# vkit-dev/vkit-ocr-model-adaptive-scaling

Measured on AMD Instinct MI355X. Metric: images/sec fwd+bwd @1024x1024 bf16 (train step: rough+precise passes, losses, backward, clip, AdamW), higher is better.
Workload: dtype bf16

## Files before the change

### include/vkas.h

```cpp
#ifndef VKAS_H
#define VKAS_H

#include <stddef.h>
#include <stdint.h>

#ifdef __cplusplus
extern "C" {
#endif

#define VKAS_F32 0
#define VKAS_BF16 1
#define VKAS_F16 2

#define VKAS_OK 0
#define VKAS_E_ARG (-1)
#define VKAS_E_LAUNCH (-2)

#define VKAS_EPI_NONE 0
#define VKAS_EPI_GELU 1
#define VKAS_EPI_SCALE_RES 2
#define VKAS_EPI_DGELU 3
#define VKAS_EPI_ADD 4
#define VKAS_EPI_PATCH 5
#define VKAS_EPI_HEAD 6

const char* vkas_last_error(void);
int vkas_abi_version(void);

typedef struct vkas_conv_geom {
  int B, Hin, Win, Hout, Wout;
  int Cp;
  int ldx;
  int KH, KW, stride, pad;
} vkas_conv_geom;

typedef struct vkas_head_desc {
  int n_heads, pw;
  int n0[4], np[4], c[4], oc[4];
  const float* params;
  float* stats;
  float* proj;
} vkas_head_desc;

typedef struct vkas_epilogue {
  int mode;
  const float* bias;
  void* out;  long ldo;
  void* out2; long ldo2;
  const void* aux; long ldaux;
  const float* colscale;
  const float* rowscale;
  int rows_per_image;
  int patch;
  int patch_Hs, patch_Ws, patch_Cp;
  vkas_head_desc head;
} vkas_epilogue;

int vkas_pack_conv_weight(const float* w, void* out, int N, int C, int KH, int KW, int Np, int Cp, int mode,
                          int dtype, void* stream);
int vkas_pack_conv_weight_slice(const float* w, void* out, int N, int C, int KH, int KW, int Np, int Cp, int mode,
                                int n_off, int Nt, int dtype, void* stream);
int vkas_unpack_conv_wgrad(const float* gw, float* grad, int N, int C, int KH, int KW, int Np, int Cp,
                           int accumulate, void* stream);
int vkas_accumulate_many(int count, const float* const* src, float* const* dst, const int* n, void* stream);
int vkas_finalize_many(int count, const float* const* partial, const long* P, const int* n, const int* ldp,
                       float* const* out, const int* accumulate, void* stream);
long vkas_layernorm_bwd_parts(long M, int Cp);
long vkas_scale_res_bwd_parts(long M, int Cp);
long vkas_dwconv7x7_wgrad_parts(int B, int H, int W, int Cp, int dtype);
int vkas_pad_vector(const float* v, float* out, int n, int np, void* stream);
size_t vkas_dw_weight_elems(int Cp);
int vkas_pack_dw_weight(const float* w, float* out, int C, int Cp, int flip, void* stream);
int vkas_unpack_dw_wgrad(const float* gw, float* grad, int C, int Cp, int accumulate, void* stream);
int vkas_image_nchw_to_nhwc8(const float* img, void* out, int B, int C, int H, int W, int dtype, void* stream);
int vkas_nhwc_to_nchw_f32(const void* x, long ld, float* out, int B, int H, int W, int C, int dtype, void* stream);
int vkas_nchw_f32_to_nhwc(const float* g, void* out, long ld, int B, int H, int W, int C, int Cp, int dtype, void* stream);

int vkas_conv_gemm_fwd(const void* x, const vkas_conv_geom* g, const void* Bw, int Np, const vkas_epilogue* epi,
                       int dtype, void* stream);
int vkas_conv_gemm_wgrad(const void* x, const vkas_conv_geom* g, const void* dy, long lddy, int Np, float* gw,
                         float* gb, int dtype, void* stream);
int vkas_conv_gemm_wgrad_ordered(const void* x, const vkas_conv_geom* g, const void* dy, long lddy, int Np, float* gw,
                                 int dtype, void* stream);
int vkas_conv_gemm_wgrad_gelu(const void* x, const vkas_conv_geom* g, const void* dy, long lddy, int Np, float* gw,
                              float* gb, int dtype, void* stream);

size_t vkas_upconv5_fold_elems(int Np, int Cp, int f, int transposed);
int vkas_upconv5_fold(const float* w, void* out, int N, int C, int Np, int Cp, int f, int transposed, int dtype, void* stream);
int vkas_upconv5_fwd(const void* x, const vkas_conv_geom* g, int f, const void* Bf, int Np, const float* bias, void* out,
                     long ldo, int dtype, void* stream);
int vkas_upconv5_dgrad(const void* dy, long lddy, const vkas_conv_geom* g, int f, const void* Bt, int Np, void* dx, long lddx,
                       int dtype, void* stream);
size_t vkas_upconv5_wgrad_ws_bytes(int B, int H, int W, int Np);
int vkas_upconv5_wgrad(const void* x, const vkas_conv_geom* g, int f, const void* dy, long lddy, int Np, void* ws,
                       size_t ws_bytes, float* gwf, float* gb, int dtype, void* stream);
int vkas_upconv5_unfold_wgrad(const float* gwf, float* dw, int N, int C, int Np, int Cp, int f, int accumulate, void* stream);

size_t vkas_mlp_chain_image_elems(int C);
int vkas_mlp_chain_pack(const float* w1, const float* w2, const float* b1, int C, int mode, void* img, int dtype,
                        void* stream);
int vkas_mlp_chain_fwd(const void* yn, long ldyn, const void* img, const float* b2, const void* x, long ldx,
                       const float* colscale, const float* rowscale, int rows_per_image, void* h, long ldh, void* z,
                       long ldz, void* out, long ldo, long M, int C, int dtype, void* stream);
int vkas_mlp_chain_ln_fwd(const void* y, long ldy, const float* ln_gamma, const float* ln_beta, void* yn, long ldyn,
                          float* stats, const void* img, const float* b2, const void* x, long ldx, const float* colscale,
                          const float* rowscale, int rows_per_image, void* h, long ldh, void* z, long ldz, void* out,
                          long ldo, long M, int C, int dtype, void* stream);
int vkas_mlp_chain_bwd(const void* dz, long lddz, const void* img_t, const void* h, long ldh, void* dh, long lddh,
                       void* dyn, long lddyn, long M, int C, int dtype, void* stream);
int vkas_conv_gemm_tile(int wgrad, long M, int Np, int K);
int vkas_conv_gemm_kernel_id(int wgrad, const vkas_conv_geom* g, int Np, long lddy, int head_width);
typedef struct vkas_gemm_switches {
  int nt_tile, tn_tile;
  int nt_ring;
  int nt_noslab, nt_nobuf, tn_nobuf, tn_noslab, tn_no96;
} vkas_gemm_switches;
typedef struct vkas_gemm_plan_info {
  int kernel_id, family, bn, ring, buf, head, pw, nobias, xg;
  long grid_m, grid_n, tiles, splits, rows, a_bytes, b_bytes;
  unsigned grid;
  char name[44];
} vkas_gemm_plan_info;
int vkas_conv_gemm_plan(int wgrad, const vkas_conv_geom* g, int Np, long lddy, int head_width, int flags, int has_gb,
                        const vkas_gemm_switches* sw, vkas_gemm_plan_info* out);
int vkas_colsum(const void* y, long ld, long M, int Np, float* out, int accumulate, float* ws, size_t ws_bytes,
                int dtype, void* stream);
size_t vkas_colsum_ws_bytes(long M, int Np);

int vkas_dwconv7x7_fwd(const void* x, long ldx, const float* w, const float* bias, const void* addend, long ldadd,
                       void* y, long ldy, int B, int H, int W, int Cp, int dtype, void* stream);
int vkas_dwconv7x7_wgrad(const void* x, long ldx, const void* dy, long lddy, float* gw, float* gb, float* ws,
                         size_t ws_bytes, int B, int H, int W, int Cp, int dtype, void* stream);
size_t vkas_dwconv7x7_wgrad_ws_bytes(int B, int H, int W, int Cp);

int vkas_layernorm_fwd(const void* x, long ldx, const float* gamma, const float* beta, void* y, long ldy,
                       float* stats, long M, int C, int Cp, int act_gelu, int dtype, void* stream);
int vkas_layernorm_bwd(const void* x, long ldx, const float* gamma, const float* beta, const float* stats,
                       const void* dy, long lddy, void* dx, long lddx, float* dgamma, float* dbeta, float* ws,
                       size_t ws_bytes, long M, int C, int Cp, int act_gelu, int dtype, void* stream);
size_t vkas_layernorm_bwd_ws_bytes(long M, int Cp);

int vkas_pack_head_params(const float* gamma, const float* beta, const float* wproj, const float* bproj, int C, int oc,
                          int pw, float* out, void* stream);
int vkas_head_tail_fwd(const void* z, long ldz, const vkas_head_desc* hd, long M, int dtype, void* stream);
int vkas_head_rows_fwd(const void* T, const float* bias, const vkas_head_desc* hd, void* z, int B, int h, int W2, int Nt,
                       int seg_rows, int dtype, void* stream);
int vkas_head_tail_bwd(const void* z, long ldz, const vkas_head_desc* hd, const float* const* dproj, void* dz, long lddz,
                       float* dparams, float* ws, size_t ws_bytes, long M, int dtype, void* stream);
size_t vkas_head_tail_bwd_ws_bytes(long M, int pw);

int vkas_scale_res_bwd(const void* dout, long lddo, const void* z, long ldz, const float* colscale,
                       const float* rowscale, int rows_per_image, void* dz, long lddz, float* dscale, float* dbias,
                       float* ws, size_t ws_bytes, long M, int Cp, int dtype, void* stream);
size_t vkas_scale_res_bwd_ws_bytes(long M, int Cp);

int vkas_resize_fwd(const void* x, long ldx, void* y, long ldy, int B, int Hin, int Win, int Hout, int Wout,
                    int Cp, int mode, int accumulate, int dtype, void* stream);
int vkas_resize2x_x_fwd(const void* x, long ldx, void* y, long ldy, int B, int H, int Win, int Cp, int dtype, void* stream);
int vkas_resize_bwd(const void* dy, long lddy, void* dx, long lddx, int B, int Hin, int Win, int Hout, int Wout,
                    int Cp, int mode, int accumulate, int dtype, void* stream);
size_t vkas_resize_bwd_ws_bytes(int B, int Hin, int Win, int Hout, int Wout, int Cp);
int vkas_resize_bwd_ws(const void* dy, long lddy, void* dx, long lddx, float* ws, size_t ws_bytes, int B, int Hin, int Win,
                       int Hout, int Wout, int Cp, int mode, int accumulate, int dtype, void* stream);

int vkas_upconv_adj(const void* dz, long lddz, void* E, int B, int h, int w, int N, int dtype, void* stream);
size_t vkas_upconv_adj_colsum_ws_bytes(int B, int h, int w, int N);
int vkas_upconv_adj_colsum(const void* dz, long lddz, void* E, int B, int h, int w, int N, float* out, int accumulate, float* ws,
                           size_t ws_bytes, int dtype, void* stream);
int vkas_upconv_adj_colsum_seg(const void* dz, long lddz, void* E, int B, int h, int w, int N, float* out, int accumulate,
                               float* ws, size_t ws_bytes, int dtype, void* stream, int seg_rows);
int vkas_upconv_adj_unpack_wgrad(const float* gE, float* gwp, int N, int Cp, void* stream);

int vkas_adaptive_avgpool_fwd(const void* x, long ldx, void* y, long ldy, int B, int H, int W, int s, int Cp,
                              int dtype, void* stream);
int vkas_adaptive_avgpool_bwd(const void* dy, long lddy, void* dx, long lddx, int B, int H, int W, int s, int Cp,
                              int accumulate, int dtype, void* stream);

#define VKAS_PPM_MAX_BRANCHES 4
#define VKAS_PPM_MAX_SCALE 16
#define VKAS_PPM_MAX_CELLS 256
#define VKAS_PPM_MAX_C 2048
#define VKAS_PPM_MAX_CB 512
long vkas_ppm_row_groups(int B, int nb, const int* scales);
int vkas_ppm_pool_fwd(const void* x, long ldx, void* cat, long ldcat, float* rowsum, int B, int H, int W, int C, int Cb,
                      int nb, const int* scales, int dtype, void* stream);
int vkas_ppm_rows_fwd(const float* rowsum, const float* const* params, void* pooled, void* lin, float* stats, void* act, int B,
                      int H, int W, int C, int Cb, int nb, const int* scales, int dtype, void* stream);
int vkas_ppm_resize_fwd(const void* act, void* cat, long ldcat, int B, int H, int W, int C, int Cb, int nb, const int* scales,
                        int dtype, void* stream);
int vkas_ppm_resize_bwd_x(const void* dcat, long lddcat, float* tx, int B, int H, int W, int C, int Cb, int nb,
                          const int* scales, int dtype, void* stream);
int vkas_ppm_rows_bwd(const float* tx, const float* const* params, const void* lin, const float* stats, void* dz,
                      float* partial, float* dp, int B, int H, int W, int C, int Cb, int nb, const int* scales, int dtype,
                      void* stream);
int vkas_ppm_param_grads(const void* dz, const void* pooled, const float* partial, float* const* grads, const int* accumulate,
                         int B, int C, int Cb, int nb, const int* scales, int dtype, void* stream);
int vkas_ppm_pool_bwd(const void* dcat, long lddcat, const float* dp, void* dx, long lddx, int B, int H, int W, int C, int Cb,
                      int nb, const int* scales, int dtype, void* stream);

int vkas_copy_channels(const void* x, long ldx, void* y, long ldy, long M, int Cp, int accumulate, int dtype,
                       void* stream);
int vkas_copy_channel_range(const void* x, long ldx, int c_src, void* y, long ldy, int c_dst, long M, int C,
                            int zero_tail, int dtype, void* stream);
int vkas_softplus_fwd(const float* x, float* y, long n, void* stream);
int vkas_softplus_bwd(const float* x, const float* dy, float* dx, long n, void* stream);

typedef struct vkas_rough_loss_cfg {
  float focal_factor, dice_factor, l1_factor, score_min, height_min;
  float focal_alpha, focal_gamma;
  float out_scale;
} vkas_rough_loss_cfg;
int vkas_rough_loss_fwd(const float* mask_feat, const float* height_feat, const float* gt_mask,
                        const float* gt_score, int B, int H, int W, int up, int left, int CH, int CW,
                        const vkas_rough_loss_cfg* cfg, double* sums, float* loss, void* stream);
int vkas_rough_loss_bwd(const float* mask_feat, const float* height_feat, const float* gt_mask,
                        const float* gt_score, int B, int H, int W, int up, int left, int CH, int CW,
                        const vkas_rough_loss_cfg* cfg, const double* sums, const float* dloss, float* d_mask_feat,
                        float* d_height_feat, void* stream);

typedef struct vkas_precise_loss_cfg {
  float pos_l2, neg_l2, offset_l1, reg_l1, angle_ce, dist_l1, loss_factor;
  float smooth_beta;
  float out_scale;
} vkas_precise_loss_cfg;
int vkas_points_margin(const int64_t* py, const int64_t* px, long n, int H, int W, int64_t* margin, void* stream);
typedef struct vkas_precise_loss_extra_cfg {
  float mask_focal, prob_l1, prob_wahr;
  float prob_l1_beta;
  float wahr_gamma;
  float focal_alpha, focal_gamma;
} vkas_precise_loss_extra_cfg;
#define VKAS_PRECISE_LOSS_SUMS 16
int vkas_precise_loss_fwd(const float* prob, const float* offset, const float* angle, const float* dist,
                          const float* gt_score, const float* gt_mask, const int64_t* py, const int64_t* px,
                          const float* gt_offsets, const float* gt_angles, const float* gt_dists, int B, int H,
                          int W, int up, int left, int CH, int CW, int P, const vkas_precise_loss_cfg* cfg,
                          const float* mask_feat, const vkas_precise_loss_extra_cfg* ex, double* sums, float* loss,
                          void* stream);
int vkas_precise_loss_bwd(const float* prob, const float* offset, const float* angle, const float* dist,
                          const float* gt_score, const float* gt_mask, const int64_t* py, const int64_t* px,
                          const float* gt_offsets, const float* gt_angles, const float* gt_dists, int B, int H,
                          int W, int up, int left, int CH, int CW, int P, const vkas_precise_loss_cfg* cfg,
                          const float* mask_feat, const vkas_precise_loss_extra_cfg* ex, const double* sums,
                          const float* dloss, float* d_prob, float* d_offset, float* d_angle, float* d_dist,
                          float* d_mask_feat, void* stream);

#define VKAS_LOSS_FOCAL 0
#define VKAS_LOSS_DICE 1
#define VKAS_LOSS_L1 2
#define VKAS_LOSS_SMOOTH_L1 3
#define VKAS_LOSS_L2 4
#define VKAS_LOSS_WAHR 5
int vkas_elementwise_loss_fwd(int kind, const float* pred, const float* gt, const float* mask, long n, float p0, float p1,
                              float eps, double* sums, float* loss, void* stream);
int vkas_elementwise_loss_bwd(int kind, const float* pred, const float* gt, const float* mask, long n, float p0, float p1,
                              float eps, const double* sums, const float* dloss, float* dpred, void* stream);
int vkas_cross_entropy_fwd(const float* logits, const void* target, int hard, long rows, int classes, double* sums,
                           float* loss, void* stream);
int vkas_cross_entropy_bwd(const float* logits, const void* target, int hard, long rows, int classes, const float* dloss,
                           float* dlogits, void* stream);

int vkas_points_prepare(const long* py, const long* px, int B, int P, int H, int W, int* map, int* pix, long Mp, void* stream);
int vkas_points_gather_rows(const void* z, long ldz, int c0, int Ns, const float* stats, const float* const* dproj,
                            int n_heads, long M, const int* pix, long Mp, void* zs, float* stats_s, float* dproj_s,
                            int dtype, void* stream);
int vkas_points_gather_patches(const void* x, long ldx, int Cp, int B, int H, int W, const int* pix, long Mp, void* xs,
                               int dtype, void* stream);
int vkas_points_gather_patches_up2(const void* x, long ldx, int Cp, int B, int h, int w, const int* pix, long Mp, void* xs,
                                   int dtype, void* stream);
int vkas_points_scatter3x3(const float* D, const int* pix, const int* map, long Mp, int B, int H, int W, int Cp, void* dx,
                           long lddx, int dtype, void* stream);
int vkas_points_scatter3x3_low(const float* D, const int* pix, const int* map, long Mp, int B, int h, int w, int Cp, void* dx,
                               long lddx, int dtype, void* stream);

int vkas_points_scatter_vec8(const float* src, const int* pix, long Mp, float* dst, void* stream);
int vkas_points_gather_vec8(const float* src, const int* pix, long Mp, float* dst, void* stream);

typedef struct {
  const float* w;
  void* out;
  long total;
  int kind, N, C, KH, KW, Np, Cp, mode, n_off, Nt, dtype;
} vkas_pack_desc;
int vkas_pack_many(const vkas_pack_desc* descs, const int* block_start, int count, int total_blocks, void* stream);
int vkas_pack_many_blocks(const vkas_pack_desc* d);

int vkas_rough_postprocess(const float* mask_logit, const float* height, int B, int H, int W, const int* valid_h,
                           const int* valid_w, float mask_thr, float height_min, unsigned char* out_mask,
                           float* out_height, void* stream);
int vkas_precise_postprocess(const float* prob_logit, const float* offset, const float* angle, const float* dist, int B,
                             int H, int W, const int* valid_h, const int* valid_w, float* out_prob, float* out_offset,
                             float* out_angle, float* out_dist, void* stream);
long vkas_char_polygons_workspace_bytes(int B, int H, int W, int size);
int vkas_char_polygons(const float* prob, const float* offset, const float* angle, const float* dist, int B, int H, int W,
                       int size, float thr, float scale_y, float scale_x, void* workspace, size_t workspace_bytes,
                       int* count, int* points, float* probs, float* quads, void* stream);
int vkas_char_label_maps(const int* rows, const int* count, int B, int K, int h, int w, int up, int left, int CH, int CW,
                         float k, int* owner, float* mask, float* height, float* score, void* stream);
long long vkas_quad_match_workspace_bytes(int B, int M, int N, int max_pairs);
int vkas_quad_match(const int* gt_rows, const int* gt_count, const int* pred_rows, const int* pred_count, int B, int M, int N,
                    double iou_thr, int max_pairs, void* workspace, size_t workspace_bytes, int* gt_match, int* pred_match,
                    double* gt_iou, long long* stats, int* rounds, void* stream);
long long vkas_quad_match_ranked_workspace_bytes(int B, int M, int N, int T, int max_pairs);
int vkas_quad_match_ranked(const int* gt_rows, const int* gt_count, const unsigned char* gt_care, const int* pred_rows,
                           const int* pred_count, const float* probs, int B, int M, int N, const double* iou_thrs, int T,
                           double cover_thr, int max_pairs, void* workspace, size_t workspace_bytes, int* pred_match,
                           unsigned char* pred_state, int* gt_match, double* pred_iou, unsigned char* covered,
                           long long* stats, long long* dc_stats, int* rounds, void* stream);
int vkas_quad_rows(const double* quads, const unsigned char* valid, int B, int K, int* rows, void* stream);
long long vkas_quad_nms_workspace_bytes(int B, int K, int max_pairs);
int vkas_quad_nms(const int* rows, const int* count, const float* probs, int B, int K, double iou_thr, int max_pairs,
                  void* workspace, size_t workspace_bytes, unsigned char* keep, int* suppressor, long long* stats, int* rounds,
                  void* stream);
long long vkas_line_match_workspace_bytes(int B, int M, int N, int max_pairs);
int vkas_line_match(const int* gt_rows, const int* gt_count, const unsigned char* gt_care, const int* pred_rows,
                    const int* pred_count, int B, int M, int N, int tr_q8, int tp_q8, double cover_thr, int max_pairs,
                    void* workspace, size_t workspace_bytes, unsigned char* gt_kind, int* gt_group, unsigned char* pred_kind,
                    int* pred_group, long long* stats, int* rounds, void* stream);
long long vkas_ribbon_match_workspace_bytes(int B, int M, int N, int max_pairs);
int vkas_ribbon_match(const int* gt_rows, const int* gt_count, const unsigned char* gt_care, const int* gt_segs, int Sg,
                      const int* pred_rows, const int* pred_count, const int* pred_segs, int Sp, int B, int M, int N, int tr_q8,
                      int tp_q8, double cover_thr, int max_pairs, void* workspace, size_t workspace_bytes,
                      unsigned char* gt_kind, int* gt_group, unsigned char* pred_kind, int* pred_group, long long* stats,
                      int* rounds, void* stream);
long long vkas_quad_lines_workspace_bytes(int B, int K);
int vkas_quad_lines(const int* rows, const int* count, int B, int K, int gap_q4, int cross_q4, int ratio_q4, void* workspace,
                    size_t workspace_bytes, int* line, int* order, long long* table, long long* stats, void* stream);
long long vkas_text_regions_workspace_bytes(int B, int H, int W, int max_regions);
int vkas_text_regions(const unsigned char* mask, const float* height, int B, int H, int W, int max_regions, void* workspace,
                      long long workspace_bytes, int* count, int* labels, int* boxes, int* areas, int* valid, float* medians,
                      void* stream);
int vkas_resample_pack_u8(const unsigned char* src, int Hs, int Ws, const int* placements, int n, unsigned char* page,
                          int Hp, int Wp, void* stream);
int vkas_pack_region_labels(const int* labels, int Hl, int Wl, int valid_h, int valid_w, int Hs, int Ws,
                            const int* placements, const int* region_ids, int n, int fdf, int* out, int Hq, int Wq,
                            void* stream);
int vkas_resample_pack_u8_multi(const unsigned char* arena, long long arena_bytes, const long long* sources, int S,
                                const int* rows, int n, const int* page_start, unsigned char* pages, int Q, int Hp, int Wp,
                                void* stream);
int vkas_pack_region_labels_multi(const int* label_arena, long long label_words, const long long* label_sources, int S,
                                  const int* rows, int n, const int* page_start, int fdf, int* out, int Q, int Hq, int Wq,
                                  void* stream);
int vkas_region_moments(const int* labels, int B, int H, int W, int max_regions, long long* moments, void* stream);
int vkas_region_extents(const int* labels, int B, int H, int W, int max_regions, const int* dirs, int* extents,
                        void* stream);
int vkas_warp_pack_u8(const unsigned char* src, int Hs, int Ws, const long long* warps, int n, unsigned char* page, int Hp,
                      int Wp, void* stream);
int vkas_warp_region_labels(const int* labels, int Hl, int Wl, int valid_h, int valid_w, int Hs, int Ws,
                            const long long* warps, const int* region_ids, int n, int fdf, int* out, int Hq, int Wq,
                            void* stream);
int vkas_crop_warp_f32(const unsigned char* arena, long long arena_bytes, const long long* sources, int S,
                       const long long* rows, int B, float* out, int H, int W, void* stream);
int vkas_quad_strips_u8(const unsigned char* arena, long long arena_bytes, const long long* sources, int S,
                        const long long* rows, int n, int h, unsigned char* out, long long out_bytes, void* stream);
long long vkas_spine_strips_workspace_bytes(long long columns);
int vkas_spine_columns(const long long* table, int n, long long knots_total, int h, long long* columns,
                       long long columns_cap, void* stream);
int vkas_spine_strips_u8(const unsigned char* arena, long long arena_bytes, const long long* sources, int S,
                         const long long* table, int n, long long knots_total, int h, void* ws, long long ws_bytes,
                         unsigned char* out, long long out_bytes, void* stream);

int vkas_l2norm_sq(const float* g, long n, double* sumsq, void* stream);
int vkas_adamw_step(float* p, const float* g, float* m, float* v, long n, const double* sumsq, float max_norm,
                    float grad_scale, float lr, float beta1, float beta2, float eps, float weight_decay, int step,
                    void* stream);

#ifdef __cplusplus
}
#endif
#endif
```

### vkit_ocr_model_adaptive_scaling_amd/_lib.py

```python
import ctypes
import os
from ctypes import POINTER, Structure, c_char, c_char_p, c_double, c_float, c_int, c_int64, c_long, c_longlong, c_size_t, c_uint, c_void_p

_HERE = os.path.dirname(os.path.abspath(__file__))
LIB_PATH = os.environ.get('VKAS_LIB_PATH') or os.path.join(_HERE, 'libvkas.so')

F32, BF16, F16 = 0, 1, 2
EPI_NONE, EPI_GELU, EPI_SCALE_RES, EPI_DGELU, EPI_ADD, EPI_PATCH, EPI_HEAD = range(7)
LOSS_FOCAL, LOSS_DICE, LOSS_L1, LOSS_SMOOTH_L1, LOSS_L2 = range(5)
LOSS_WAHR = 5
PRECISE_LOSS_SUMS = 16


class ConvGeom(Structure):
    _fields_ = [('B', c_int), ('Hin', c_int), ('Win', c_int), ('Hout', c_int), ('Wout', c_int), ('Cp', c_int),
                ('ldx', c_int), ('KH', c_int), ('KW', c_int), ('stride', c_int), ('pad', c_int)]


class HeadDesc(Structure):
    _fields_ = [('n_heads', c_int), ('pw', c_int), ('n0', c_int * 4), ('np', c_int * 4), ('c', c_int * 4),
                ('oc', c_int * 4), ('params', c_void_p), ('stats', c_void_p), ('proj', c_void_p)]


class Epilogue(Structure):
    _fields_ = [('mode', c_int), ('bias', c_void_p), ('out', c_void_p), ('ldo', c_long), ('out2', c_void_p),
                ('ldo2', c_long), ('aux', c_void_p), ('ldaux', c_long), ('colscale', c_void_p),
                ('rowscale', c_void_p), ('rows_per_image', c_int), ('patch', c_int), ('patch_Hs', c_int),
                ('patch_Ws', c_int), ('patch_Cp', c_int), ('head', HeadDesc)]


class GemmSwitches(Structure):
    _fields_ = [('nt_tile', c_int), ('tn_tile', c_int), ('nt_ring', c_int), ('nt_noslab', c_int), ('nt_nobuf', c_int),
                ('tn_nobuf', c_int), ('tn_noslab', c_int), ('tn_no96', c_int)]

    def __init__(self, nt_ring=-1, **kw):
        super().__init__(nt_ring=nt_ring, **kw)


class GemmPlanInfo(Structure):
    _fields_ = [(n, c_int) for n in ('kernel_id', 'family', 'bn', 'ring', 'buf', 'head', 'pw', 'nobias', 'xg')] + \
               [(n, c_long) for n in ('grid_m', 'grid_n', 'tiles', 'splits', 'rows', 'a_bytes', 'b_bytes')] + \
               [('grid', c_uint), ('name', c_char * 44)]


class PackDesc(Structure):
    _fields_ = [('w', c_void_p), ('out', c_void_p), ('total', c_long), ('kind', c_int), ('N', c_int), ('C', c_int),
                ('KH', c_int), ('KW', c_int), ('Np', c_int), ('Cp', c_int), ('mode', c_int), ('n_off', c_int),
                ('Nt', c_int), ('dtype', c_int)]


class RoughLossCfg(Structure):
    _fields_ = [('focal_factor', c_float), ('dice_factor', c_float), ('l1_factor', c_float), ('score_min', c_float),
                ('height_min', c_float), ('focal_alpha', c_float), ('focal_gamma', c_float), ('out_scale', c_float)]


class PreciseLossCfg(Structure):
    _fields_ = [('pos_l2', c_float), ('neg_l2', c_float), ('offset_l1', c_float), ('reg_l1', c_float),
                ('angle_ce', c_float), ('dist_l1', c_float), ('loss_factor', c_float), ('smooth_beta', c_float),
                ('out_scale', c_float)]


class PreciseLossExtraCfg(Structure):
    _fields_ = [('mask_focal', c_float), ('prob_l1', c_float), ('prob_wahr', c_float), ('prob_l1_beta', c_float),
                ('wahr_gamma', c_float), ('focal_alpha', c_float), ('focal_gamma', c_float)]


class VkasError(RuntimeError):
    pass


if not os.path.exists(LIB_PATH):
    raise ImportError(
        f'{LIB_PATH} not found: build the HIP kernels first (python -c "import __graft_entry__ as g; g.build()" '
        f'or make -C {os.path.join(_HERE, "csrc")}).  There is no CPU fallback.')

lib = ctypes.CDLL(LIB_PATH)

_P = c_void_p
_SIGS = {
    'vkas_last_error': (c_char_p, []),
    'vkas_abi_version': (c_int, []),
    'vkas_pack_conv_weight': (c_int, [_P, _P, c_int, c_int, c_int, c_int, c_int, c_int, c_int, c_int, _P]),
    'vkas_pack_conv_weight_slice': (c_int, [_P, _P, c_int, c_int, c_int, c_int, c_int, c_int, c_int, c_int, c_int, c_int, _P]),
    'vkas_unpack_conv_wgrad': (c_int, [_P, _P, c_int, c_int, c_int, c_int, c_int, c_int, c_int, _P]),
    'vkas_accumulate_many': (c_int, [c_int, POINTER(c_void_p), POINTER(c_void_p), POINTER(c_int), _P]),
    'vkas_finalize_many': (c_int, [c_int, POINTER(c_void_p), POINTER(c_long), POINTER(c_int), POINTER(c_int), POINTER(c_void_p),
                                   POINTER(c_int), _P]),
    'vkas_layernorm_bwd_parts': (c_long, [c_long, c_int]),
    'vkas_scale_res_bwd_parts': (c_long, [c_long, c_int]),
    'vkas_dwconv7x7_wgrad_parts': (c_long, [c_int, c_int, c_int, c_int, c_int]),
    'vkas_pad_vector': (c_int, [_P, _P, c_int, c_int, _P]),
    'vkas_dw_weight_elems': (c_size_t, [c_int]),
    'vkas_pack_dw_weight': (c_int, [_P, _P, c_int, c_int, c_int, _P]),
    'vkas_unpack_dw_wgrad': (c_int, [_P, _P, c_int, c_int, c_int, _P]),
    'vkas_image_nchw_to_nhwc8': (c_int, [_P, _P, c_int, c_int, c_int, c_int, c_int, _P]),
    'vkas_nhwc_to_nchw_f32': (c_int, [_P, c_long, _P, c_int, c_int, c_int, c_int, c_int, _P]),
    'vkas_nchw_f32_to_nhwc': (c_int, [_P, _P, c_long, c_int, c_int, c_int, c_int, c_int, c_int, _P]),
    'vkas_conv_gemm_fwd': (c_int, [_P, POINTER(ConvGeom), _P, c_int, POINTER(Epilogue), c_int, _P]),
    'vkas_conv_gemm_wgrad': (c_int, [_P, POINTER(ConvGeom), _P, c_long, c_int, _P, _P, c_int, _P]),
    'vkas_conv_gemm_wgrad_ordered': (c_int, [_P, POINTER(ConvGeom), _P, c_long, c_int, _P, c_int, _P]),
    'vkas_conv_gemm_wgrad_gelu': (c_int, [_P, POINTER(ConvGeom), _P, c_long, c_int, _P, _P, c_int, _P]),
    'vkas_upconv5_fold_elems': (c_size_t, [c_int, c_int, c_int, c_int]),
    'vkas_upconv5_fold': (c_int, [_P, _P, c_int, c_int, c_int, c_int, c_int, c_int, c_int, _P]),
    'vkas_upconv5_fwd': (c_int, [_P, POINTER(ConvGeom), c_int, _P, c_int, _P, _P, c_long, c_int, _P]),
    'vkas_upconv5_dgrad': (c_int, [_P, c_long, POINTER(ConvGeom), c_int, _P, c_int, _P, c_long, c_int, _P]),
    'vkas_upconv5_wgrad_ws_bytes': (c_size_t, [c_int, c_int, c_int, c_int]),
    'vkas_upconv5_wgrad': (c_int, [_P, POINTER(ConvGeom), c_int, _P, c_long, c_int, _P, c_size_t, _P, _P, c_int, _P]),
    'vkas_upconv5_unfold_wgrad': (c_int, [_P, _P, c_int, c_int, c_int, c_int, c_int, c_int, _P]),
    'vkas_mlp_chain_image_elems': (c_size_t, [c_int]),
    'vkas_mlp_chain_pack': (c_int, [_P, _P, _P, c_int, c_int, _P, c_int, _P]),
    'vkas_mlp_chain_fwd': (c_int, [_P, c_long, _P, _P, _P, c_long, _P, _P, c_int, _P, c_long, _P, c_long, _P, c_long,
                                   c_long, c_int, c_int, _P]),
    'vkas_mlp_chain_ln_fwd': (c_int, [_P, c_long, _P, _P, _P, c_long, _P, _P, _P, _P, c_long, _P, _P, c_int, _P, c_long, _P,
                                      c_long, _P, c_long, c_long, c_int, c_int, _P]),
    'vkas_mlp_chain_bwd': (c_int, [_P, c_long, _P, _P, c_long, _P, c_long, _P, c_long, c_long, c_int, c_int, _P]),
    'vkas_conv_gemm_tile': (c_int, [c_int, c_long, c_int, c_int]),
    'vkas_conv_gemm_kernel_id': (c_int, [c_int, POINTER(ConvGeom), c_int, c_long, c_int]),
    'vkas_conv_gemm_plan': (c_int, [c_int, POINTER(ConvGeom), c_int, c_long, c_int, c_int, c_int, POINTER(GemmSwitches),
                                    POINTER(GemmPlanInfo)]),
    'vkas_colsum': (c_int, [_P, c_long, c_long, c_int, _P, c_int, _P, c_size_t, c_int, _P]),
    'vkas_colsum_ws_bytes': (c_size_t, [c_long, c_int]),
    'vkas_dwconv7x7_fwd': (c_int, [_P, c_long, _P, _P, _P, c_long, _P, c_long, c_int, c_int, c_int, c_int, c_int, _P]),
    'vkas_dwconv7x7_wgrad': (c_int, [_P, c_long, _P, c_long, _P, _P, _P, c_size_t, c_int, c_int, c_int, c_int, c_int, _P]),
    'vkas_dwconv7x7_wgrad_ws_bytes': (c_size_t, [c_int, c_int, c_int, c_int]),
    'vkas_layernorm_fwd': (c_int, [_P, c_long, _P, _P, _P, c_long, _P, c_long, c_int, c_int, c_int, c_int, _P]),
    'vkas_layernorm_bwd': (c_int, [_P, c_long, _P, _P, _P, _P, c_long, _P, c_long, _P, _P, _P, c_size_t, c_long, c_int,
                                   c_int, c_int, c_int, _P]),
    'vkas_layernorm_bwd_ws_bytes': (c_size_t, [c_long, c_int]),
    'vkas_pack_head_params': (c_int, [_P, _P, _P, _P, c_int, c_int, c_int, _P, _P]),
    'vkas_head_tail_fwd': (c_int, [_P, c_long, _P, c_long, c_int, _P]),
    'vkas_head_rows_fwd': (c_int, [_P, _P, POINTER(HeadDesc), _P, c_int, c_int, c_int, c_int, c_int, c_int, _P]),
    'vkas_resize2x_x_fwd': (c_int, [_P, c_long, _P, c_long, c_int, c_int, c_int, c_int, c_int, _P]),
    'vkas_points_gather_patches_up2': (c_int, [_P, c_long, c_int, c_int, c_int, c_int, _P, c_long, _P, c_int, _P]),
    'vkas_head_tail_bwd': (c_int, [_P, c_long, POINTER(HeadDesc), POINTER(c_void_p), _P, c_long, _P, _P, c_size_t, c_long, c_int, _P]),
    'vkas_head_tail_bwd_ws_bytes': (c_size_t, [c_long, c_int]),
    'vkas_scale_res_bwd': (c_int, [_P, c_long, _P, c_long, _P, _P, c_int, _P, c_long, _P, _P, _P, c_size_t, c_long,
                                   c_int, c_int, _P]),
    'vkas_scale_res_bwd_ws_bytes': (c_size_t, [c_long, c_int]),
    'vkas_resize_fwd': (c_int, [_P, c_long, _P, c_long, c_int, c_int, c_int, c_int, c_int, c_int, c_int, c_int, c_int, _P]),
    'vkas_resize_bwd': (c_int, [_P, c_long, _P, c_long, c_int, c_int, c_int, c_int, c_int, c_int, c_int, c_int, c_int, _P]),
    'vkas_resize_bwd_ws_bytes': (c_size_t, [c_int, c_int, c_int, c_int, c_int, c_int]),
    'vkas_resize_bwd_ws': (c_int, [_P, c_long, _P, c_long, _P, c_size_t, c_int, c_int, c_int, c_int, c_int, c_int, c_int, c_int,
                                   c_int, _P]),
    'vkas_upconv_adj': (c_int, [_P, c_long, _P, c_int, c_int, c_int, c_int, c_int, _P]),
    'vkas_upconv_adj_colsum_ws_bytes': (c_size_t, [c_int, c_int, c_int, c_int]),
    'vkas_upconv_adj_colsum': (c_int, [_P, c_long, _P, c_int, c_int, c_int, c_int, _P, c_int, _P, c_size_t, c_int, _P]),
    'vkas_upconv_adj_colsum_seg': (c_int, [_P, c_long, _P, c_int, c_int, c_int, c_int, _P, c_int, _P, c_size_t, c_int, _P, c_int]),
    'vkas_upconv_adj_unpack_wgrad': (c_int, [_P, _P, c_int, c_int, _P]),
    'vkas_adaptive_avgpool_fwd':(c_int, [_P, c_long, _P, c_long, c_int, c_int, c_int, c_int, c_int, c_int, _P]),
    'vkas_adaptive_avgpool_bwd': (c_int, [_P, c_long, _P, c_long, c_int, c_int, c_int, c_int, c_int, c_int, c_int, _P]),
    'vkas_ppm_row_groups': (c_long, [c_int, c_int, POINTER(c_int)]),
    'vkas_ppm_pool_fwd': (c_int, [_P, c_long, _P, c_long, _P] + [c_int] * 6 + [POINTER(c_int), c_int, _P]),
    'vkas_ppm_rows_fwd': (c_int, [_P, POINTER(c_void_p), _P, _P, _P, _P] + [c_int] * 6 + [POINTER(c_int), c_int, _P]),
    'vkas_ppm_resize_fwd': (c_int, [_P, _P, c_long] + [c_int] * 6 + [POINTER(c_int), c_int, _P]),
    'vkas_ppm_resize_bwd_x': (c_int, [_P, c_long, _P] + [c_int] * 6 + [POINTER(c_int), c_int, _P]),
    'vkas_ppm_rows_bwd': (c_int, [_P, POINTER(c_void_p), _P, _P, _P, _P, _P] + [c_int] * 6 + [POINTER(c_int), c_int, _P]),
    'vkas_ppm_param_grads': (c_int, [_P, _P, _P, POINTER(c_void_p), POINTER(c_int)] + [c_int] * 4 + [POINTER(c_int), c_int, _P]),
    'vkas_ppm_pool_bwd': (c_int, [_P, c_long, _P, _P, c_long] + [c_int] * 6 + [POINTER(c_int), c_int, _P]),
    'vkas_copy_channels': (c_int, [_P, c_long, _P, c_long, c_long, c_int, c_int, c_int, _P]),
    'vkas_copy_channel_range': (c_int, [_P, c_long, c_int, _P, c_long, c_int, c_long, c_int, c_int, c_int, _P]),
    'vkas_softplus_fwd': (c_int, [_P, _P, c_long, _P]),
    'vkas_softplus_bwd': (c_int, [_P, _P, _P, c_long, _P]),
    'vkas_rough_loss_fwd': (c_int, [_P, _P, _P, _P, c_int, c_int, c_int, c_int, c_int, c_int, c_int,
                                    POINTER(RoughLossCfg), _P, _P, _P]),
    'vkas_rough_loss_bwd': (c_int, [_P, _P, _P, _P, c_int, c_int, c_int, c_int, c_int, c_int, c_int,
                                    POINTER(RoughLossCfg), _P, _P, _P, _P, _P]),
    'vkas_points_margin': (c_int, [_P, _P, c_long, c_int, c_int, _P, _P]),
    'vkas_precise_loss_fwd': (c_int, [_P] * 11 + [c_int] * 8 + [POINTER(PreciseLossCfg), _P, POINTER(PreciseLossExtraCfg),
                                                                  _P, _P, _P]),
    'vkas_precise_loss_bwd': (c_int, [_P] * 11 + [c_int] * 8 + [POINTER(PreciseLossCfg), _P, POINTER(PreciseLossExtraCfg)]
                              + [_P] * 8),
    'vkas_elementwise_loss_fwd': (c_int, [c_int, _P, _P, _P, c_long, c_float, c_float, c_float, _P, _P, _P]),
    'vkas_elementwise_loss_bwd': (c_int, [c_int, _P, _P, _P, c_long, c_float, c_float, c_float, _P, _P, _P, _P]),
    'vkas_cross_entropy_fwd': (c_int, [_P, _P, c_int, c_long, c_int, _P, _P, _P]),
    'vkas_cross_entropy_bwd': (c_int, [_P, _P, c_int, c_long, c_int, _P, _P, _P]),
    'vkas_points_prepare': (c_int, [_P, _P, c_int, c_int, c_int, c_int, _P, _P, c_long, _P]),
    'vkas_points_gather_rows': (c_int, [_P, c_long, c_int, c_int, _P, _P, c_int, c_long, _P, c_long, _P, _P, _P, c_int, _P]),
    'vkas_points_gather_patches': (c_int, [_P, c_long, c_int, c_int, c_int, c_int, _P, c_long, _P, c_int, _P]),
    'vkas_points_scatter3x3': (c_int, [_P, _P, _P, c_long, c_int, c_int, c_int, c_int, _P, c_long, c_int, _P]),
    'vkas_points_scatter3x3_low': (c_int, [_P, _P, _P, c_long, c_int, c_int, c_int, c_int, _P, c_long, c_int, _P]),
    'vkas_points_scatter_vec8': (c_int, [_P, _P, c_long, _P, _P]),
    'vkas_points_gather_vec8': (c_int, [_P, _P, c_long, _P, _P]),
    'vkas_pack_many': (c_int, [_P, _P, c_int, c_int, _P]),
    'vkas_pack_many_blocks': (c_int, [_P]),
    'vkas_rough_postprocess': (c_int, [_P, _P, c_int, c_int, c_int, _P, _P, c_float, c_float, _P, _P, _P]),
    'vkas_precise_postprocess': (c_int, [_P, _P, _P, _P, c_int, c_int, c_int, _P, _P, _P, _P, _P, _P, _P]),
    'vkas_char_polygons_workspace_bytes': (c_long, [c_int, c_int, c_int, c_int]),
    'vkas_char_polygons': (c_int, [_P, _P, _P, _P, c_int, c_int, c_int, c_int, c_float, c_float, c_float, _P, c_size_t,
                                   _P, _P, _P, _P, _P]),
    'vkas_char_label_maps': (c_int, [_P, _P, c_int, c_int, c_int, c_int, c_int, c_int, c_int, c_int, c_float, _P, _P, _P, _P,
                                     _P]),
    'vkas_quad_match_workspace_bytes': (c_longlong, [c_int, c_int, c_int, c_int]),
    'vkas_quad_match': (c_int, [_P, _P, _P, _P, c_int, c_int, c_int, c_double, c_int, _P, c_size_t, _P, _P, _P, _P, _P, _P]),
    'vkas_quad_match_ranked_workspace_bytes': (c_longlong, [c_int, c_int, c_int, c_int, c_int]),
    'vkas_quad_match_ranked': (c_int, [_P, _P, _P, _P, _P, _P, c_int, c_int, c_int, _P, c_int, c_double, c_int, _P, c_size_t,
                                       _P, _P, _P, _P, _P, _P, _P, _P, _P]),
    'vkas_quad_rows': (c_int, [_P, _P, c_int, c_int, _P, _P]),
    'vkas_quad_nms_workspace_bytes': (c_longlong, [c_int, c_int, c_int]),
    'vkas_quad_nms': (c_int, [_P, _P, _P, c_int, c_int, c_double, c_int, _P, c_size_t, _P, _P, _P, _P, _P]),
    'vkas_line_match_workspace_bytes': (c_longlong, [c_int, c_int, c_int, c_int]),
    'vkas_line_match': (c_int, [_P, _P, _P, _P, _P, c_int, c_int, c_int, c_int, c_int, c_double, c_int, _P, c_size_t, _P, _P, _P,
                                _P, _P, _P, _P]),
    'vkas_ribbon_match_workspace_bytes': (c_longlong, [c_int, c_int, c_int, c_int]),
    'vkas_ribbon_match': (c_int, [_P, _P, _P, _P, c_int, _P, _P, _P, c_int, c_int, c_int, c_int, c_int, c_int, c_double, c_int,
                                  _P, c_size_t, _P, _P, _P, _P, _P, _P, _P]),
    'vkas_quad_lines_workspace_bytes': (c_longlong, [c_int, c_int]),
    'vkas_quad_lines': (c_int, [_P, _P, c_int, c_int, c_int, c_int, c_int, _P, c_size_t, _P, _P, _P, _P, _P]),
    'vkas_text_regions_workspace_bytes': (c_longlong, [c_int, c_int, c_int, c_int]),
    'vkas_text_regions': (c_int, [_P, _P, c_int, c_int, c_int, c_int, _P, c_longlong, _P, _P, _P, _P, _P, _P, _P]),
    'vkas_resample_pack_u8': (c_int, [_P, c_int, c_int, _P, c_int, _P, c_int, c_int, _P]),
    'vkas_pack_region_labels': (c_int, [_P, c_int, c_int, c_int, c_int, c_int, c_int, _P, _P, c_int, c_int, _P, c_int, c_int,
                                        _P]),
    'vkas_resample_pack_u8_multi': (c_int, [_P, c_longlong, _P, c_int, _P, c_int, _P, _P, c_int, c_int, c_int, _P]),
    'vkas_pack_region_labels_multi': (c_int, [_P, c_longlong, _P, c_int, _P, c_int, _P, c_int, _P, c_int, c_int, c_int, _P]),
    'vkas_region_moments': (c_int, [_P, c_int, c_int, c_int, c_int, _P, _P]),
    'vkas_region_extents': (c_int, [_P, c_int, c_int, c_int, c_int, _P, _P, _P]),
    'vkas_warp_pack_u8': (c_int, [_P, c_int, c_int, _P, c_int, _P, c_int, c_int, _P]),
    'vkas_warp_region_labels': (c_int, [_P, c_int, c_int, c_int, c_int, c_int, c_int, _P, _P, c_int, c_int, _P, c_int, c_int,
                                        _P]),
    'vkas_crop_warp_f32': (c_int, [_P, c_longlong, _P, c_int, _P, c_int, _P, c_int, c_int, _P]),
    'vkas_quad_strips_u8': (c_int, [_P, c_longlong, _P, c_int, _P, c_int, c_int, _P, c_longlong, _P]),
    'vkas_spine_strips_workspace_bytes': (c_longlong, [c_longlong]),
    'vkas_spine_columns': (c_int, [_P, c_int, c_longlong, c_int, _P, c_longlong, _P]),
    'vkas_spine_strips_u8': (c_int, [_P, c_longlong, _P, c_int, _P, c_int, c_longlong, c_int, _P, c_longlong, _P, c_longlong,
                                     _P]),
    'vkas_l2norm_sq':(c_int, [_P, c_long, _P, _P]),
    'vkas_adamw_step': (c_int, [_P, _P, _P, _P, c_long, _P, c_float, c_float, c_float, c_float, c_float, c_float,
                                c_float, c_int, _P]),
}

EXPORTS = tuple(_SIGS)

for _name, (_res, _args) in _SIGS.items():
    _fn = getattr(lib, _name)
    _fn.restype = _res
    _fn.argtypes = _args


def check(rc: int, what: str = ''):
    if rc != 0:
# ... 3 lines not shown
```

### vkit_ocr_model_adaptive_scaling_amd/csrc/gemm_api.hip

```cpp
#include <stdlib.h>
#include <string.h>

#include "gemm_parts.h"
#include "gemm_plan.h"

int vkas_gemm_nt_simple(const void*, const vkas_conv_geom*, const void*, int, const vkas_epilogue*, int, hipStream_t);
int vkas_gemm_tn_simple(const void*, const vkas_conv_geom*, const void*, long, int, float*, float*, int, int, hipStream_t);
int vkas_gemm_nt_mfma_bf16(const void*, const vkas_conv_geom*, const void*, int, const vkas_epilogue*, hipStream_t);
int vkas_gemm_tn_mfma_bf16(const void*, const vkas_conv_geom*, const void*, long, int, float*, float*, int, hipStream_t);
int vkas_gemm_nt_mfma_f16(const void*, const vkas_conv_geom*, const void*, int, const vkas_epilogue*, hipStream_t);
int vkas_gemm_tn_mfma_f16(const void*, const vkas_conv_geom*, const void*, long, int, float*, float*, int, hipStream_t);

static thread_local char g_err[512] = "";

void vkas_set_error(const char* fmt, ...) {
  va_list ap;
  va_start(ap, fmt);
  vsnprintf(g_err, sizeof(g_err), fmt, ap);
  va_end(ap);
}

extern "C" const char* vkas_last_error(void) { return g_err; }
extern "C" int vkas_abi_version(void) { return 1; }

// ... 60 lines not shown
  int rc = vkas_check_geom("vkas_conv_gemm_fwd", x, g, Np);
  if (rc) return rc;
  rc = vkas_check_epilogue("vkas_conv_gemm_fwd", epi, Np);
  if (rc) return rc;
  VKAS_CHECK(Bw && vkas_aligned16(Bw), "vkas_conv_gemm_fwd: weights null/misaligned");
  if (epi->mode == VKAS_EPI_PATCH)
    VKAS_CHECK((long)g->B * g->Hout * g->Wout == (long)g->B * epi->patch_Hs * epi->patch_Ws || g->B == 0,
               "vkas_conv_gemm_fwd: patch grid does not match the GEMM rows");
  if (epi->mode == VKAS_EPI_HEAD)
    VKAS_CHECK((dtype == VKAS_BF16 || dtype == VKAS_F16) && !force_simple() && (long)g->B * g->Hout * g->Wout >= 16384,
               "vkas_conv_gemm_fwd: the fused head epilogue exists for the 16-bit MFMA kernels (M >= 16384) only");
  if (g->KH == 1 && g->KW == 3)
    VKAS_CHECK((dtype == VKAS_BF16 || dtype == VKAS_F16) && !force_simple() && epi->mode == VKAS_EPI_NONE,
               "vkas_conv_gemm_fwd: the 1x3 row convolution exists for the 16-bit MFMA kernels with the plain epilogue only");
  if (dtype == VKAS_BF16 && !force_simple()) return vkas_gemm_nt_mfma_bf16(x, g, Bw, Np, epi, vkas_stream(stream));
  if (dtype == VKAS_F16 && !force_simple()) return vkas_gemm_nt_mfma_f16(x, g, Bw, Np, epi, vkas_stream(stream));
  return vkas_gemm_nt_simple(x, g, Bw, Np, epi, dtype, vkas_stream(stream));
}

extern "C" int vkas_conv_gemm_plan(int wgrad, const vkas_conv_geom* g, int Np, long lddy, int head_width, int flags, int has_gb,
                                   const vkas_gemm_switches* sw, vkas_gemm_plan_info* out) {
  VKAS_CHECK(g && out, "vkas_conv_gemm_plan: null argument");
  vkas_gemm_plan_info o = {};
  if (!sw && force_simple()) {
    snprintf(o.name, sizeof(o.name), wgrad ? "gemm_tn_simple" : "gemm_nt_simple");
  } else if (wgrad) {
    const vkas_tn_plan p = vkas_plan_tn(*g, Np, lddy, flags, has_gb != 0, sw ? *sw : *vkas_gemm_env_switches());
    o = {vkas_tn_kernel_id(p), p.family, p.tile, 0, p.buf, 0, p.pw, p.nobias, p.xg, 0, 0, p.tiles, p.splits, p.rows, p.x_bytes, p.dy_bytes, p.grid, ""};
    const char* t = p.tile == 128 ? "2,2,4" : (p.tile == 192 ? "2,4,6" : (p.tile == 224 ? "2,4,7" : "4,2,6"));
    if (p.family == VKAS_TN_SLAB) snprintf(o.name, sizeof(o.name), "conv3x3_wgrad_slab_kernel<%d>", p.tile / 16);
    else snprintf(o.name, sizeof(o.name), "gemm_tn_mfma_kernel<%s,4>", t);
  } else {
    const vkas_nt_plan p = vkas_plan_nt(*g, Np, head_width, sw ? *sw : *vkas_gemm_env_switches());
    const long tiles = p.grid_m * p.grid_n;
    o = {vkas_nt_kernel_id(p), p.family, p.bn, p.ring, p.buf, p.head, 0, 0, 0, p.grid_m, p.grid_n, tiles, 1, 0, p.a_bytes, p.b_bytes, (unsigned)tiles, ""};
    if (p.family == VKAS_NT_SLAB && p.kh == 1) snprintf(o.name, sizeof(o.name), "conv1x3_slab_mfma_kernel<%d>", p.bn / 32);
    else if (p.family == VKAS_NT_SLAB) snprintf(o.name, sizeof(o.name), "conv3x3_slab_mfma_kernel<%d,%d>", p.bn / 32, (int)p.head);
    else if (p.family == VKAS_NT_RING) snprintf(o.name, sizeof(o.name), "gemm_nt_ring_kernel<%d>", p.ring);
    else snprintf(o.name, sizeof(o.name), "gemm_nt_mfma_kernel<%s,4,%d>", p.family == VKAS_NT_REG128 ? "2,2" : "4,2", p.bn / 32);
  }
  *out = o;
  return VKAS_OK;
}

extern "C" int vkas_conv_gemm_tile(int wgrad, long M, int Np, int K) {
  if (force_simple()) return 0;
  const vkas_gemm_switches& sw = *vkas_gemm_env_switches();
  return wgrad ? vkas_tn_tile_rule(M, Np, K, sw) : vkas_nt_tile_rule(M, Np, sw);
}

extern "C" int vkas_conv_gemm_kernel_id(int wgrad, const vkas_conv_geom* g, int Np, long lddy, int head_width) {
  vkas_gemm_plan_info o;
  return g && vkas_conv_gemm_plan(wgrad, g, Np, lddy, head_width, 0, 0, nullptr, &o) == VKAS_OK ? o.kernel_id : 0;
}

static int conv_gemm_wgrad(const char* who, const void* x, const vkas_conv_geom* g, const void* dy, long lddy, int Np,
                           float* gw, float* gb, int x_gelu, int dtype, void* stream) {
  int rc = vkas_check_geom(who, x, g, Np);
  if (rc) return rc;
  VKAS_CHECK(dy && vkas_aligned16(dy) && lddy >= Np && lddy % 8 == 0, "%s: bad dy (lddy=%ld)", who, lddy);
  VKAS_CHECK(gw, "%s: null gw", who);
  VKAS_CHECK(!(g->KH == 1 && g->KW == 3), "%s: the 1x3 row convolution has no weight-gradient kernel", who);
  if (dtype == VKAS_BF16 && !force_simple())
    return vkas_gemm_tn_mfma_bf16(x, g, dy, lddy, Np, gw, gb, x_gelu, vkas_stream(stream));
  if (dtype == VKAS_F16 && !force_simple())
    return vkas_gemm_tn_mfma_f16(x, g, dy, lddy, Np, gw, gb, x_gelu, vkas_stream(stream));
  return vkas_gemm_tn_simple(x, g, dy, lddy, Np, gw, gb, x_gelu, dtype, vkas_stream(stream));
}

extern "C" int vkas_conv_gemm_wgrad(const void* x, const vkas_conv_geom* g, const void* dy, long lddy, int Np,
                                    float* gw, float* gb, int dtype, void* stream) {
  return conv_gemm_wgrad("vkas_conv_gemm_wgrad", x, g, dy, lddy, Np, gw, gb, 0, dtype, stream);
}

extern "C" int vkas_conv_gemm_wgrad_ordered(const void* x, const vkas_conv_geom* g, const void* dy, long lddy, int Np,
                                            float* gw, int dtype, void* stream) {
  return conv_gemm_wgrad("vkas_conv_gemm_wgrad_ordered", x, g, dy, lddy, Np, gw, nullptr, 2, dtype, stream);
}

extern "C" int vkas_conv_gemm_wgrad_gelu(const void* x, const vkas_conv_geom* g, const void* dy, long lddy, int Np,
                                         float* gw, float* gb, int dtype, void* stream) {
  return conv_gemm_wgrad("vkas_conv_gemm_wgrad_gelu", x, g, dy, lddy, Np, gw, gb, 1, dtype, stream);
}

namespace {
static inline long cs_rows_per_block(long M) { long r = vkas_cdiv(M > 0 ? M : 1, 1024); return r < 32 ? 32 : r; }

template <typename T>
__global__ __launch_bounds__(256) void colsum_partial_kernel(const T* __restrict__ y, long ld, long M, int Np,
                                                             long rows_per_block, float* __restrict__ partial,
                                                             int ldp) {
  const int nvec = Np >> 3;
  const int lanes_r = 256 / nvec > 0 ? 256 / nvec : 1;
  const int v = threadIdx.x % nvec;
  const int rl = threadIdx.x / nvec;
  float acc[8] = {0, 0, 0, 0, 0, 0, 0, 0};
  const long mbeg = (long)blockIdx.x * rows_per_block;
  const long mend = mbeg + rows_per_block < M ? mbeg + rows_per_block : M;
  if (rl < lanes_r) {
    for (long m = mbeg + rl; m < mend; m += lanes_r) {
      float t[8];
      load8(y + m * ld + v * 8, t);
#pragma unroll
      for (int i = 0; i < 8; ++i) acc[i] += t[i];
    }
  }
  __shared__ float red[256 * 8];
#pragma unroll
  for (int i = 0; i < 8; ++i) red[threadIdx.x * 8 + i] = acc[i];
  __syncthreads();
  if (rl == 0) {
    for (int r = 1; r < lanes_r; ++r)
#pragma unroll
      for (int i = 0; i < 8; ++i) acc[i] += red[(r * nvec + v) * 8 + i];
    float* dst = partial + (long)blockIdx.x * ldp + v * 8;
#pragma unroll
    for (int i = 0; i < 8; ++i) dst[i] = acc[i];
  }
}
}

__global__ __launch_bounds__(256) void vkas_colreduce_finalize_kernel(const float* __restrict__ partial, long P, int n,
                                                                      int ldp, float* __restrict__ out,
                                                                      int accumulate) {
  __shared__ float red[16][17];
  const int cl = threadIdx.x & 15, rl = threadIdx.x >> 4;
  const int c = blockIdx.x * 16 + cl;
  float acc[8];
#pragma unroll
  for (int i = 0; i < 8; ++i) acc[i] = 0.f;
  if (c < n) {
    long p = rl;
    for (; p + 7 * 16 < P; p += 8 * 16) {
#pragma unroll
      for (int i = 0; i < 8; ++i) acc[i] += partial[(p + 16 * i) * ldp + c];
    }
    for (; p < P; p += 16) acc[0] += partial[p * ldp + c];
  }
  red[rl][cl] = ((acc[0] + acc[1]) + (acc[2] + acc[3])) + ((acc[4] + acc[5]) + (acc[6] + acc[7]));
  __syncthreads();
  if (rl == 0 && c < n) {
    float s = 0.f;
#pragma unroll
    for (int r = 0; r < 16; ++r) s += red[r][cl];
    out[c] = accumulate ? out[c] + s : s;
  }
}

struct FinalizeMany {
  const float* partial[8];
  float* out[8];
  long P[8];
  int n[8], ldp[8], accumulate[8], first[9];
};
__global__ __launch_bounds__(256) void vkas_finalize_many_kernel(FinalizeMany a) {
  __shared__ float red[16][17];
  int k = 0;
#pragma unroll
  for (int i = 1; i < 8; ++i) k += ((int)blockIdx.x >= a.first[i]) ? 1 : 0;
  const float* __restrict__ partial = a.partial[k];
  const long P = a.P[k];
  const int n = a.n[k], ldp = a.ldp[k];
  const int cl = threadIdx.x & 15, rl = threadIdx.x >> 4;
  const int c = ((int)blockIdx.x - a.first[k]) * 16 + cl;
  float acc[8];
#pragma unroll
  for (int i = 0; i < 8; ++i) acc[i] = 0.f;
  if (c < n) {
    long p = rl;
    for (; p + 7 * 16 < P; p += 8 * 16) {
#pragma unroll
      for (int i = 0; i < 8; ++i) acc[i] += partial[(p + 16 * i) * ldp + c];
    }
    for (; p < P; p += 16) acc[0] += partial[p * ldp + c];
  }
  red[rl][cl] = ((acc[0] + acc[1]) + (acc[2] + acc[3])) + ((acc[4] + acc[5]) + (acc[6] + acc[7]));
  __syncthreads();
  if (rl == 0 && c < n) {
    float s = 0.f;
#pragma unroll
    for (int r = 0; r < 16; ++r) s += red[r][cl];
    float* out = a.out[k];
    out[c] = a.accumulate[k] ? out[c] + s : s;
  }
}

extern "C" int vkas_finalize_many(int count, const float* const* partial, const long* P, const int* n, const int* ldp,
                                  float* const* out, const int* accumulate, void* stream) {
  VKAS_CHECK(count >= 0 && count <= 8 && (count == 0 || (partial && P && n && ldp && out && accumulate)),
             "vkas_finalize_many: bad arguments (count=%d)", count);
  if (count == 0) return VKAS_OK;
  FinalizeMany a;
  int blocks = 0;
  for (int k = 0; k < 8; ++k) {
    a.first[k] = blocks;
    if (k < count) {
      VKAS_CHECK(partial[k] && out[k] && P[k] >= 0 && n[k] >= 0 && ldp[k] >= n[k], "vkas_finalize_many: bad reduction %d", k);
      a.partial[k] = partial[k];
      a.out[k] = out[k];
      a.P[k] = P[k];
      a.n[k] = n[k];
      a.ldp[k] = ldp[k];
      a.accumulate[k] = accumulate[k];
      blocks += (int)vkas_cdiv(n[k], 16);
    } else {
      a.partial[k] = nullptr; a.out[k] = nullptr; a.P[k] = 0; a.n[k] = 0; a.ldp[k] = 0; a.accumulate[k] = 0;
    }
  }
  a.first[8] = blocks;
  for (int k = count; k < 8; ++k) a.first[k] = blocks;
  if (blocks == 0) return VKAS_OK;
  vkas_finalize_many_kernel<<<(unsigned)blocks, 256, 0, vkas_stream(stream)>>>(a);
  VKAS_LAUNCH_CHECK("finalize_many");
  return VKAS_OK;
}

int vkas_colreduce_finalize(const float* partial, long P, int n, int ldp, float* out, int accumulate,
                            hipStream_t st) {
  vkas_colreduce_finalize_kernel<<<(unsigned)vkas_cdiv(n, 16), 256, 0, st>>>(partial, P, n, ldp, out, accumulate);
  VKAS_LAUNCH_CHECK("colreduce_finalize");
  return VKAS_OK;
}

extern "C" size_t vkas_colsum_ws_bytes(long M, int Np) {
  return (size_t)vkas_cdiv(M > 0 ? M : 1, cs_rows_per_block(M)) * (size_t)Np * sizeof(float);
}

extern "C" int vkas_colsum(const void* y, long ld, long M, int Np, float* out, int accumulate, float* ws,
                           size_t ws_bytes, int dtype, void* stream) {
  VKAS_CHECK(y && out && ws, "vkas_colsum: null pointer");
  VKAS_CHECK(Np > 0 && Np % 8 == 0, "vkas_colsum: Np=%d must be a positive multiple of 8", Np);
  VKAS_CHECK(ld >= Np && ld % 8 == 0 && vkas_aligned16(y), "vkas_colsum: bad ld/alignment");
  VKAS_CHECK(ws_bytes >= vkas_colsum_ws_bytes(M, Np), "vkas_colsum: workspace too small");
  if (M <= 0) {
    if (!accumulate) (void)hipMemsetAsync(out, 0, Np * sizeof(float), vkas_stream(stream));
    return VKAS_OK;
  }
  const long rpb = cs_rows_per_block(M);
  const long P = vkas_cdiv(M, rpb);
  VKAS_DISPATCH_DTYPE(dtype, "vkas_colsum", {
    for (int c0 = 0; c0 < Np; c0 += 2048) {
      const int n = Np - c0 < 2048 ? Np - c0 : 2048;
      colsum_partial_kernel<T><<<(unsigned)P, 256, 0, vkas_stream(stream)>>>((const T*)y + c0, ld, M, n, rpb, ws + c0, Np);
    }
  })
  VKAS_LAUNCH_CHECK("colsum_partial");
  return vkas_colreduce_finalize(ws, P, Np, Np, out, accumulate, vkas_stream(stream));
}
```

### vkit_ocr_model_adaptive_scaling_amd/csrc/mlp_chain.hip

```cpp
#include <stdlib.h>

#include <type_traits>

#include "vkas_common.h"

namespace {

typedef __attribute__((address_space(3))) void* lds_void_ptr;

constexpr int MODE_FWD = 0, MODE_BWD = 1;

#ifndef CHAIN_ABL
#define CHAIN_ABL 0
#endif
constexpr int ABL = CHAIN_ABL;

__host__ __device__ constexpr int chain_ka(int KS) { return ((KS + 1) / 2) * 64; }
__host__ __device__ constexpr int chain_img_elems(int KS) { return 32 * chain_ka(KS) + KS * 32 * 32 + 512; }

template <typename T, typename V4>
__device__ __forceinline__ V4 chain_gelu4(const V4& h) {
  const f32x2 a = gelu2_t<T>(f32x2{(float)h[0], (float)h[1]}), b = gelu2_t<T>(f32x2{(float)h[2], (float)h[3]});
  V4 o;
  o[0] = (T)a.x; o[1] = (T)a.y; o[2] = (T)b.x; o[3] = (T)b.y;
  return o;
}
template <typename T, typename V4>
__device__ __forceinline__ V4 chain_dgelu4(const V4& h, const f32x4& d) {
  const f32x2 a = f32x2{d[0], d[1]} * dgelu2_t<T>(f32x2{(float)h[0], (float)h[1]});
  const f32x2 b = f32x2{d[2], d[3]} * dgelu2_t<T>(f32x2{(float)h[2], (float)h[3]});
  V4 o;
  o[0] = (T)a.x; o[1] = (T)a.y; o[2] = (T)b.x; o[3] = (T)b.y;
  return o;
}

template <typename T>
__global__ void mlp_chain_pack_kernel(const float* __restrict__ w1, const float* __restrict__ w2,
                                      const float* __restrict__ b1, int C, int HID, int KS, int mode, T* __restrict__ img) {
  const int KA = chain_ka(KS);
  const int pieces = chain_img_elems(KS) / 8;
  const long idx = (long)blockIdx.x * blockDim.x + threadIdx.x;
  const int nchunks = HID / 32;
  if (idx >= (long)nchunks * pieces) return;
  const int j = (int)(idx / pieces);
  int p = (int)(idx - (long)j * pieces);
  float v[8];
  const int a_pieces = 32 * KA / 8;
  const int b_pieces = KS * 32 * 32 / 8;
  if (p >= a_pieces + b_pieces) {
    const int q = p - a_pieces - b_pieces;
    float4 bv = make_float4(0.f, 0.f, 0.f, 0.f);
    if (q < 8 && mode == 0 && b1) bv = *reinterpret_cast<const float4*>(b1 + j * 32 + q * 4);
    *reinterpret_cast<float4*>(img + idx * 8) = bv;
    return;
  }
  if (p < a_pieces) {
    const int s = p / 256, rem = p - s * 256;
    const int h = rem >> 3, cpos = rem & 7;
    const int c = cpos ^ (h & 7);
    const int k0 = s * 64 + c * 8;
    const int hid = j * 32 + h;
#pragma unroll
    for (int i = 0; i < 8; ++i) {
      const int k = k0 + i;
      v[i] = k < C ? (mode == 0 ? w1[(long)hid * C + k] : w2[(long)k * HID + hid]) : 0.f;
    }
  } else {
    p -= a_pieces;
    const int R = p >> 3, cpos = p & 7;
    const int c = cpos ^ (R & 7);
    const int n = R * 2 + (c >> 2), g = c & 3;
#pragma unroll
    for (int q = 0; q < 8; ++q) {
      const int hid = j * 32 + (q >> 2) * 16 + g * 4 + (q & 3);
      v[q] = n < C ? (mode == 0 ? w2[(long)n * HID + hid] : w1[(long)hid * C + n]) : 0.f;
    }
  }
  store8(img + idx * 8, v);
}

struct ChainArgs {
  const void* a;
  long lda;
  const void* img;
  void* mid_out;
  long ldm;
  const void* mid_in;
  long ldmi;
  const float* bias_b;
  const void* res;
  long ldres;
  const float* colscale;
  const float* rowscale;
  int rows_per_image;
  void* z;
  long ldz;
  void* out;
  long ldo;
  long M;
  int C, HID;
  const float* ln_gamma;
  const float* ln_beta;
  void* ln_out;
  long ldln;
  float* ln_stats;
};

template <typename T> struct Frag;
template <> struct Frag<bf16_t> { typedef bf16x8 v8; typedef bf16x4 v4; };
template <> struct Frag<f16_t> { typedef f16x8 v8; typedef f16x4 v4; };

__device__ __forceinline__ f32x4 mfma16(bf16x8 a, bf16x8 b, f32x4 c) {
  return __builtin_amdgcn_mfma_f32_16x16x32_bf16(a, b, c, 0, 0, 0);
}
__device__ __forceinline__ f32x4 mfma16(f16x8 a, f16x8 b, f32x4 c) {
  return __builtin_amdgcn_mfma_f32_16x16x32_f16(a, b, c, 0, 0, 0);
}

template <int NTHR>
__device__ __forceinline__ void chain_layernorm_stage(const ChainArgs& p, float* lnp, int tid) {
  const int cq = p.C >> 2;
  for (int i = tid; i < 2 * cq; i += NTHR) {
    const bool hi = i >= cq;
    const int idx = hi ? i - cq : i;
    *reinterpret_cast<float4*>(lnp + (hi ? p.C : 0) + idx * 4) = *reinterpret_cast<const float4*>((hi ? p.ln_beta : p.ln_gamma) + idx * 4);
  }
}

template <typename T, int TM, int KS, typename V8, typename RowFn>
__device__ __forceinline__ void chain_layernorm_rows(V8 (&xf)[TM][KS], const ChainArgs& p, RowFn mrow, int g, const float* lnp) {
  const int C = p.C;
  float mean[TM], rstd[TM];
#pragma unroll
  for (int i = 0; i < TM; ++i) {
    float s = 0.f;
#pragma unroll
    for (int ks = 0; ks < KS; ++ks)
#pragma unroll
      for (int e = 0; e < 8; ++e) s += (float)xf[i][ks][e];
    s += __shfl_xor(s, 16, 64);
    s += __shfl_xor(s, 32, 64);
    mean[i] = s / (float)C;
    float q = 0.f;
#pragma unroll
    for (int ks = 0; ks < KS; ++ks) {
      if (ks * 32 + g * 8 < C) {
#pragma unroll
        for (int e = 0; e < 8; ++e) {
          const float d = (float)xf[i][ks][e] - mean[i];
          q += d * d;
        }
      }
    }
    q += __shfl_xor(q, 16, 64);
    q += __shfl_xor(q, 32, 64);
    rstd[i] = rsqrtf(q / (float)C + 1e-6f);
  }
  T* Y = reinterpret_cast<T*>(p.ln_out);
#pragma unroll
  for (int ks = 0; ks < KS; ++ks) {
    const int k = ks * 32 + g * 8;
    const bool k_ok = k < C;
    float gv[8], bv[8];
    load8(lnp + (k_ok ? k : 0), gv);
    load8(lnp + C + (k_ok ? k : 0), bv);
#pragma unroll
    for (int i = 0; i < TM; ++i) {
      const long m = mrow(i);
      const bool ok = k_ok && m < p.M;
      V8 o;
#pragma unroll
      for (int e = 0; e < 8; ++e) o[e] = ok ? (T)(((float)xf[i][ks][e] - mean[i]) * rstd[i] * gv[e] + bv[e]) : (T)0.f;
      xf[i][ks] = o;
      if (Y && ok) *reinterpret_cast<V8*>(Y + m * p.ldln + k) = o;
    }
  }
  if (p.ln_stats && g == 0) {
#pragma unroll
    for (int i = 0; i < TM; ++i) {
      const long m = mrow(i);
      if (m < p.M) {
        p.ln_stats[2 * m] = mean[i];
        p.ln_stats[2 * m + 1] = rstd[i];
      }
    }
  }
}

template <typename T, int KS, int TM, int MODE, int MINB>
__global__ __launch_bounds__(256, MINB) void mlp_chain_kernel(ChainArgs p) {
  typedef typename Frag<T>::v8 v8;
  typedef typename Frag<T>::v4 v4;
  constexpr int NT2 = 2 * KS;
#ifdef CHAIN_OLD_SCHED
  constexpr bool HOIST = false;
#else
  constexpr bool HOIST = KS >= 4;
#endif
  constexpr int KA = chain_ka(KS);
  constexpr int IMG = chain_img_elems(KS);
  constexpr int NI = IMG * 2 / 1024;
  constexpr int ROWS = TM * 16;
  constexpr int STG = ROWS * 64;
  constexpr int NF = ROWS / 8;
  constexpr int PE = KS * 32 + 8;
  constexpr int LDS_MAIN = 2 * IMG + 4 * STG, LDS_EPI = 4 * ROWS * PE;
  constexpr int LDS_ELEMS = LDS_MAIN > LDS_EPI ? LDS_MAIN : LDS_EPI;
  static_assert((IMG * 2) % 1024 == 0, "chunk image must be whole 1-KB DMA pieces");
  __shared__ __attribute__((aligned(1024))) T lds[LDS_ELEMS];
  typedef __attribute__((address_space(3))) T lds_T;
  const int tid = threadIdx.x;
  const int lane = tid & 63;
  const int wave = __builtin_amdgcn_readfirstlane(tid >> 6);
  const int fr = lane & 15, g = lane >> 4;
  const int C = p.C;
  const long row0 = ((long)blockIdx.x * 4 + wave) * ROWS;
  const int nchunks = p.HID / 32;
  const bool full_rows = row0 + ROWS <= p.M;
  const int n_img = (NI - wave + 3) / 4;
  constexpr unsigned OOB = 0xFFFFFFF0u;

#ifdef CHAIN_BUILTIN_DMA
  const __amdgpu_buffer_rsrc_t rs_w =
      __builtin_amdgcn_make_buffer_rsrc((void*)p.img, (short)0, (int)((long)nchunks * IMG * 2), 0x00020000);
#else
  const u32x4 rs_w = vkas_make_rsrc(p.img, (unsigned)((long)nchunks * IMG * 2));
  const unsigned lds0 = vkas_lds_addr(lds);
#endif
  auto issue_chunk = [&](int j, int buf) {
#pragma unroll
    for (int q = 0; q < (NI + 3) / 4; ++q) {
// ... 600 lines not shown
        __builtin_amdgcn_sched_barrier(0);
      }
    }
    if constexpr (HAS_A) {
#pragma unroll
      for (int ab = 0; ab < NB_A; ++ab) {
        if (ab + 1 < NB_A) read_a(ab + 1, (S0 + ab + 1) & 1);
        __builtin_amdgcn_sched_barrier(0);
        mul_a(ab, (S0 + ab) & 1);
        __builtin_amdgcn_sched_barrier(0);
      }
    }
  };

  auto chunk = [&](auto no_b_c, int j) __attribute__((always_inline)) {
    constexpr bool NO_B = decltype(no_b_c)::value;
    std::integral_constant<bool, !NO_B> first_c;
    CHAIN_TR(0);
    if constexpr (CHAIN_PRIO == 1) __builtin_amdgcn_s_setprio(1);
    mfma_phase(first_c, std::true_type{}, j - 1, j);
    if constexpr (CHAIN_PRIO == 1) __builtin_amdgcn_s_setprio(0);
    CHAIN_TR(1);
    if (grp == 1) asm volatile("s_waitcnt vmcnt(0)" ::: "memory");
    asm volatile("s_waitcnt lgkmcnt(0)" ::: "memory");
    CHAIN_TR(2);
    __builtin_amdgcn_s_barrier();
    asm volatile("" ::: "memory");
    CHAIN_TR(3);
    if constexpr (CHAIN_PRIO == 2) __builtin_amdgcn_s_setprio(1);
    if (grp == 1) {
      if (!(ABL & 16)) {
        if (j + 2 < nchunks) issue_a(j + 2, wq, 4);
        if (j + 1 < nchunks) issue_b(j + 1, wq, 4);
      }
      if constexpr (MODE == MODE_BWD) {
        if ((j & 1) == 0 && j >= 2 && (j >> 1) + 1 < (nchunks + 1) / 2 && !(ABL & 1)) issue_h((j >> 1) + 1);
      }
    } else if (keep_mid && !(ABL & 1) && (j & 1) == 0 && j >= 2) {
      flush_pair((j >> 1) - 1, 64);
    }
    {
      const int e0 = (j & 1) * 32 + g * 4;
      T* stg = stg_base((j >> 1) & 1);
#pragma unroll
      for (int i = 0; i < TM; ++i) {
        const int r = (t * TM + i) * 16 + fr;
        v4 h0, h1;
        if constexpr (MODE == MODE_FWD) {
          h0[0] = (T)d[i][0][0]; h0[1] = (T)d[i][0][1]; h0[2] = (T)d[i][0][2]; h0[3] = (T)d[i][0][3];
          h1[0] = (T)d[i][1][0]; h1[1] = (T)d[i][1][1]; h1[2] = (T)d[i][1][2]; h1[3] = (T)d[i][1][3];
          if (keep_mid) {
            *reinterpret_cast<v4*>(stg + stg_off(r, e0)) = h0;
            *reinterpret_cast<v4*>(stg + stg_off(r, e0 + 16)) = h1;
          }
          const v4 g0 = (ABL & 4) ? h0 : chain_gelu4<T, v4>(h0), g1 = (ABL & 4) ? h1 : chain_gelu4<T, v4>(h1);
#pragma unroll
          for (int q = 0; q < 4; ++q) {
            own[i][q] = g0[q];
            own[i][4 + q] = g1[q];
          }
        } else {
          h0 = hq[i][0];
          h1 = hq[i][1];
          v4 o0, o1;
          if constexpr ((ABL & 4) != 0) {
#pragma unroll
            for (int q = 0; q < 4; ++q) {
              o0[q] = (T)(d[i][0][q] * (float)h0[q]);
              o1[q] = (T)(d[i][1][q] * (float)h1[q]);
            }
          } else {
            o0 = chain_dgelu4<T, v4>(h0, d[i][0]);
            o1 = chain_dgelu4<T, v4>(h1, d[i][1]);
          }
#pragma unroll
          for (int q = 0; q < 4; ++q) {
            own[i][q] = o0[q];
            own[i][4 + q] = o1[q];
          }
          *reinterpret_cast<v4*>(stg + stg_off(r, e0)) = o0;
          *reinterpret_cast<v4*>(stg + stg_off(r, e0 + 16)) = o1;
        }
        *reinterpret_cast<v8*>(exch_at(j & 1, t, i)) = own[i];
      }
    }
    if constexpr (CHAIN_PRIO == 2) __builtin_amdgcn_s_setprio(0);
    asm volatile("s_waitcnt lgkmcnt(0)" ::: "memory");
    CHAIN_TR(4);
    __builtin_amdgcn_s_barrier();
    asm volatile("" ::: "memory");
    CHAIN_TR(5);
  };
  chunk(std::true_type{}, 0);
  for (int j = 1; j < nchunks; ++j) chunk(std::false_type{}, j);
  mfma_phase(std::true_type{}, std::false_type{}, nchunks - 1, -1);
  asm volatile("s_waitcnt lgkmcnt(0)" ::: "memory");
  if (grp == 0) {
    __builtin_amdgcn_s_barrier();
    asm volatile("" ::: "memory");
    if (keep_mid && !(ABL & 1)) flush_pair((nchunks - 1) >> 1, (nchunks & 1) ? 32 : 64);
    asm volatile("s_waitcnt lgkmcnt(0)" ::: "memory");
  }
  __builtin_amdgcn_s_barrier();
  asm volatile("" ::: "memory");

  T* ep = lds + wave * (RP * PE);
  const int col0 = t * KS * 16;
#pragma unroll
  for (int n = 0; n < KS; ++n) {
    const int col = n * 16 + g * 4;
    float4 b2 = make_float4(0.f, 0.f, 0.f, 0.f);
    if constexpr (MODE == MODE_FWD) {
      if (col0 + col < C) b2 = *reinterpret_cast<const float4*>(p.bias_b + col0 + col);
    }
#pragma unroll
    for (int i = 0; i < RG; ++i) {
      v4 zq;
      zq[0] = (T)(acc[i][n][0] + b2.x);
      zq[1] = (T)(acc[i][n][1] + b2.y);
      zq[2] = (T)(acc[i][n][2] + b2.z);
      zq[3] = (T)(acc[i][n][3] + b2.w);
      *reinterpret_cast<v4*>(ep + (i * 16 + fr) * PE + col) = zq;
    }
  }
  constexpr int PCS = KS * 2;
  constexpr int RPI = 64 / PCS;
  const int piece = lane % PCS, rsub = lane / PCS;
  const int gcol = col0 + piece * 8;
  if (rsub < RPI && gcol < C) {
    float cs[8];
#pragma unroll
    for (int q = 0; q < 8; ++q) cs[q] = 0.f;
    if constexpr (MODE == MODE_FWD) load8(p.colscale + gcol, cs);
#pragma unroll 4
    for (int r = rsub; r < RP; r += RPI) {
      const long m = row0 + r;
      if (m >= p.M) break;
      const v8 zq = *reinterpret_cast<const v8*>(ep + r * PE + piece * 8);
      if constexpr (MODE == MODE_FWD) {
        if (p.z) *reinterpret_cast<v8*>(reinterpret_cast<T*>(p.z) + m * p.ldz + gcol) = zq;
        const float rs = p.rowscale ? p.rowscale[(int)(m / p.rows_per_image)] : 1.0f;
        float xr[8];
        load8(reinterpret_cast<const T*>(p.res) + m * p.ldres + gcol, xr);
#pragma unroll
        for (int q = 0; q < 8; ++q) xr[q] += rs * cs[q] * (float)zq[q];
        store8(reinterpret_cast<T*>(p.out) + m * p.ldo + gcol, xr);
      } else {
        *reinterpret_cast<v8*>(reinterpret_cast<T*>(p.out) + m * p.ldo + gcol) = zq;
      }
    }
  }
}

static int chain_ks(int C) {
  if (C <= 0 || C % 8 != 0 || C > 512) return 0;
  const int ks = (C + 31) / 32;
  return ks <= 4 ? ks : (ks <= 6 ? 6 : (ks <= 8 ? 8 : (ks <= 12 ? 12 : 16)));
}

static int chain_pair_mode() {
  static const int mode = [] {
    const char* v = getenv("VKAS_CHAIN_PAIR");
    return (v && v[0] == '0') ? 0 : 1;
  }();
  return mode;
}

template <typename T, int MODE>
static int launch_chain(const ChainArgs& a, hipStream_t st) {
  const int ks = chain_ks(a.C);
#define VKAS_CHAIN(KSV, TMV, MINB)                                                                \
  {                                                                                               \
    const long rows_per_block = 4L * TMV * 16;                                                    \
    const unsigned grid = (unsigned)vkas_cdiv(a.M, rows_per_block);                               \
    mlp_chain_kernel<T, KSV, TMV, MODE, MINB><<<grid, 256, 0, st>>>(a);                           \
  }
  switch (ks) {
    case 1: VKAS_CHAIN(1, 4, 2) break;
    case 2: VKAS_CHAIN(2, 4, 2) break;
    case 3: VKAS_CHAIN(3, 4, 2) break;
    case 4: VKAS_CHAIN(4, 2, 2) break;
    case 6: VKAS_CHAIN(6, 2, 2) break;
    case 8: VKAS_CHAIN(8, 2, 1) break;
    case 12:
      if (a.C % 16 == 0 && chain_pair_mode() != 0) {
        const unsigned grid = (unsigned)vkas_cdiv(a.M, 128);
        mlp_chain_pair_kernel<T, 12, 1, MODE><<<grid, 512, 0, st>>>(a);
      } else {
        VKAS_CHAIN(12, 2, 1)
      }
      break;
    case 16: VKAS_CHAIN(16, 2, 1) break;
    default:
      vkas_set_error("vkas_mlp_chain: C=%d is not covered (multiple of 8, <= 512)", a.C);
      return VKAS_E_ARG;
  }
#undef VKAS_CHAIN
  return VKAS_OK;
}

}

extern "C" size_t vkas_mlp_chain_image_elems(int C) {
  const int ks = chain_ks(C);
  return ks ? (size_t)(4 * C / 32) * (size_t)chain_img_elems(ks) : 0;
}

extern "C" int vkas_mlp_chain_pack(const float* w1, const float* w2, const float* b1, int C, int mode, void* img, int dtype,
                                   void* stream) {
  VKAS_CHECK(w1 && w2 && img && vkas_aligned16(img) && (mode != 0 || (b1 && vkas_aligned16(b1))),
             "vkas_mlp_chain_pack: null / misaligned pointer");
  const int ks = chain_ks(C);
  VKAS_CHECK(ks > 0, "vkas_mlp_chain_pack: C=%d is not covered (multiple of 8, <= 512)", C);
  VKAS_CHECK(mode == 0 || mode == 1, "vkas_mlp_chain_pack: mode must be 0 (forward) or 1 (backward)");
  VKAS_CHECK(dtype == VKAS_BF16 || dtype == VKAS_F16, "vkas_mlp_chain_pack: 16-bit storage types only");
  const long pieces = (long)(4 * C / 32) * (chain_img_elems(ks) / 8);
  if (dtype == VKAS_BF16)
    mlp_chain_pack_kernel<bf16_t><<<(unsigned)vkas_cdiv(pieces, 256), 256, 0, vkas_stream(stream)>>>(w1, w2, b1, C, 4 * C, ks,
                                                                                                     mode, (bf16_t*)img);
  else
    mlp_chain_pack_kernel<f16_t><<<(unsigned)vkas_cdiv(pieces, 256), 256, 0, vkas_stream(stream)>>>(w1, w2, b1, C, 4 * C, ks,
                                                                                                    mode, (f16_t*)img);
  VKAS_LAUNCH_CHECK("mlp_chain_pack");
  return VKAS_OK;
}

static int chain_check_act(const char* who, const void* p, long ld, int width) {
  VKAS_CHECK(p && vkas_aligned16(p) && ld >= width && ld % 8 == 0, "%s: bad activation operand (ld=%ld, width=%d)", who, ld, width);
  return VKAS_OK;
}

static int chain_fwd_impl(const char* who, const void* yn, long ldyn, const float* ln_gamma, const float* ln_beta, void* ln_out, long ldln,
                          float* ln_stats, const void* img, const float* b2, const void* x, long ldx, const float* colscale,
                          const float* rowscale, int rows_per_image, void* h, long ldh, void* z, long ldz, void* out, long ldo,
                          long M, int C, int dtype, void* stream) {
  VKAS_CHECK(dtype == VKAS_BF16 || dtype == VKAS_F16, "%s: 16-bit storage types only", who);
  VKAS_CHECK(chain_ks(C) > 0, "%s: C=%d is not covered (multiple of 8, <= 512)", who, C);
  VKAS_CHECK(img && b2 && colscale && vkas_aligned16(img) && vkas_aligned16(b2) && vkas_aligned16(colscale),
             "%s: null / misaligned parameter", who);
  VKAS_CHECK(M >= 0 && rows_per_image > 0, "%s: bad sizes", who);
  int rc;
  if ((rc = chain_check_act(who, yn, ldyn, C)) || (rc = chain_check_act(who, x, ldx, C)) || (rc = chain_check_act(who, out, ldo, C)))
    return rc;
  VKAS_CHECK((h == nullptr) == (z == nullptr), "%s: h and z must be given (training) or omitted (inference) together", who);
  if (h && ((rc = chain_check_act(who, h, ldh, 4 * C)) || (rc = chain_check_act(who, z, ldz, C)))) return rc;
  if (M == 0) return VKAS_OK;
  ChainArgs a = {};
  a.a = yn; a.lda = ldyn; a.img = img; a.mid_out = h; a.ldm = ldh; a.bias_b = b2; a.res = x; a.ldres = ldx;
  a.colscale = colscale; a.rowscale = rowscale; a.rows_per_image = rows_per_image; a.z = z; a.ldz = ldz; a.out = out; a.ldo = ldo;
  a.M = M; a.C = C; a.HID = 4 * C;
  a.ln_gamma = ln_gamma; a.ln_beta = ln_beta; a.ln_out = ln_out; a.ldln = ldln; a.ln_stats = ln_stats;
  rc = dtype == VKAS_BF16 ? launch_chain<bf16_t, MODE_FWD>(a, vkas_stream(stream))
                          : launch_chain<f16_t, MODE_FWD>(a, vkas_stream(stream));
  if (rc) return rc;
  VKAS_LAUNCH_CHECK("mlp_chain_fwd");
  return VKAS_OK;
}

extern "C" int vkas_mlp_chain_fwd(const void* yn, long ldyn, const void* img, const float* b2, const void* x, long ldx, const float* colscale, const float* rowscale, int rows_per_image, void* h, long ldh,
                                  void* z, long ldz, void* out, long ldo, long M, int C, int dtype, void* stream) {
  return chain_fwd_impl("vkas_mlp_chain_fwd", yn, ldyn, nullptr, nullptr, nullptr, 0, nullptr, img, b2, x, ldx, colscale, rowscale,
                        rows_per_image, h, ldh, z, ldz, out, ldo, M, C, dtype, stream);
}

extern "C" int vkas_mlp_chain_ln_fwd(const void* y, long ldy, const float* ln_gamma, const float* ln_beta, void* yn, long ldyn,
                                     float* stats, const void* img, const float* b2, const void* x, long ldx,
                                     const float* colscale, const float* rowscale, int rows_per_image, void* h, long ldh, void* z,
                                     long ldz, void* out, long ldo, long M, int C, int dtype, void* stream) {
  const char* who = "vkas_mlp_chain_ln_fwd";
  VKAS_CHECK(ln_gamma && ln_beta && vkas_aligned16(ln_gamma) && vkas_aligned16(ln_beta), "%s: null / misaligned LayerNorm parameter", who);
  VKAS_CHECK((yn == nullptr) == (h == nullptr) && (stats == nullptr) == (h == nullptr),
             "%s: yn and stats must be given (training) or omitted (inference) together with h and z", who);
  if (yn) {
    VKAS_CHECK(vkas_aligned16(yn) && ldyn >= C && ldyn % 8 == 0, "%s: bad activation operand yn (ld=%ld, width=%d)", who, ldyn, C);
  }
  return chain_fwd_impl(who, y, ldy, ln_gamma, ln_beta, yn, ldyn, stats, img, b2, x, ldx, colscale, rowscale, rows_per_image, h, ldh,
                        z, ldz, out, ldo, M, C, dtype, stream);
}

extern "C" int vkas_mlp_chain_bwd(const void* dz, long lddz, const void* img_t, const void* h, long ldh, void* dh, long lddh,
                                  void* dyn, long lddyn, long M, int C, int dtype, void* stream) {
  const char* who = "vkas_mlp_chain_bwd";
  VKAS_CHECK(dtype == VKAS_BF16 || dtype == VKAS_F16, "%s: 16-bit storage types only", who);
  VKAS_CHECK(chain_ks(C) > 0, "%s: C=%d is not covered (multiple of 8, <= 512)", who, C);
  VKAS_CHECK(img_t && vkas_aligned16(img_t) && M >= 0, "%s: bad arguments", who);
  int rc;
  if ((rc = chain_check_act(who, dz, lddz, C)) || (rc = chain_check_act(who, h, ldh, 4 * C)) || (rc = chain_check_act(who, dh, lddh, 4 * C)) ||
      (rc = chain_check_act(who, dyn, lddyn, C)))
    return rc;
  if (M == 0) return VKAS_OK;
  ChainArgs a = {};
  a.a = dz; a.lda = lddz; a.img = img_t; a.mid_out = dh; a.ldm = lddh; a.mid_in = h; a.ldmi = ldh; a.out = dyn; a.ldo = lddyn;
  a.M = M; a.C = C; a.HID = 4 * C;
  rc = dtype == VKAS_BF16 ? launch_chain<bf16_t, MODE_BWD>(a, vkas_stream(stream))
                          : launch_chain<f16_t, MODE_BWD>(a, vkas_stream(stream));
  if (rc) return rc;
  VKAS_LAUNCH_CHECK("mlp_chain_bwd");
  return VKAS_OK;
}

#ifdef CHAIN_TRACE
extern "C" int vkas_chain_trace_read(void* dst, size_t bytes) {
  return (int)hipMemcpyFromSymbol(dst, HIP_SYMBOL(vkas_chain_trace_buf), bytes < sizeof(vkas_chain_trace_buf) ? bytes : sizeof(vkas_chain_trace_buf));
}
#endif
```

### vkit_ocr_model_adaptive_scaling_amd/csrc/pack.hip

```cpp
#include "vkas_common.h"

namespace {

__device__ __forceinline__ float pack_conv_elem(const float* __restrict__ w, long i, int N, int C, int KH, int KW, int Np, int Cp,
                                                int mode, int n_off, int Nt, long& o) {
  int n, c, ky, kx;
  long r = i;
  o = i;
  if (mode == 0) {
    c = (int)(r % Cp); r /= Cp;
    kx = (int)(r % KW); r /= KW;
    ky = (int)(r % KH); r /= KH;
    n = (int)r;
    o = i + (long)n_off * KH * KW * Cp;
  } else if (mode == 1) {
    n = (int)(r % Np); r /= Np;
    o = r * Nt + n_off + n;
    kx = KW - 1 - (int)(r % KW); r /= KW;
    ky = KH - 1 - (int)(r % KH); r /= KH;
    c = (int)r;
  } else if (mode == 3) {
    c = (int)(r % Cp); r /= Cp;
    kx = (int)(r % KW); r /= KW;
    ky = (int)(r % KH); r /= KH;
    n = (int)r;
    o = (((long)ky * Nt + n_off + n) * KW + kx) * Cp + c;
  } else {
    n = (int)(r % Np); r /= Np;
    c = (int)(r % Cp); r /= Cp;
    kx = (int)(r % KW); r /= KW;
    ky = (int)r;
  }
  return (n < N && c < C) ? w[(((long)n * C + c) * KH + ky) * KW + kx] : 0.f;
}

__device__ __forceinline__ bool pack_dw_elem(const float* __restrict__ w, int i, int C, int Cp, int flip, float& v) {
  if (i < 49 * Cp) {
    const int tap = i / Cp, c = i - tap * Cp;
    const int src_tap = flip ? 48 - tap : tap;
    v = c < C ? w[(long)c * 49 + src_tap] : 0.f;
    return true;
  }
  const int j = i - 49 * Cp;
  if (j >= (Cp / 2) * 112) return false;
  const int p = j / 112, r = j - p * 112;
  const int ky = r >> 4, e = r & 15;
  const int kx = e >> 1, c = 2 * p + (e & 1);
  v = 0.f;
  if (kx < 7 && c < C) {
    const int tap = ky * 7 + kx;
    v = w[(long)c * 49 + (flip ? 48 - tap : tap)];
  }
  return true;
}

constexpr int PM_ELEMS = 2048;
__global__ __launch_bounds__(256) void pack_many_kernel(const vkas_pack_desc* __restrict__ descs,
                                                        const int* __restrict__ block_start, int count) {
  int lo = 0, hi = count;
  while (hi - lo > 1) {
    const int mid = (lo + hi) >> 1;
    if ((int)blockIdx.x >= block_start[mid]) lo = mid;
    else hi = mid;
  }
  const vkas_pack_desc d = descs[lo];
  const int lb = (int)blockIdx.x - block_start[lo];
  if (d.kind == 0 && d.mode == 1) {
    __shared__ float tile[64][33];
    const int KHW = d.KH * d.KW, J = d.C * KHW, Jp = d.Cp * KHW;
    const int tiles_n = (d.Np + 63) >> 6;
    const int jo0 = (lb / tiles_n) * 32, n0 = (lb % tiles_n) * 64;
    {
      const int l = threadIdx.x & 31, r = threadIdx.x >> 5;
      const int jo = jo0 + l;
      const int c = jo / KHW, tap = KHW - 1 - (jo - c * KHW);
      const bool j_ok = jo < Jp && c < d.C;
#pragma unroll
      for (int rr = 0; rr < 8; ++rr) {
        const int nl = rr * 8 + r, n = n0 + nl;
        tile[nl][l] = (j_ok && n < d.N) ? d.w[(long)n * J + c * KHW + tap] : 0.f;
      }
    }
    __syncthreads();
    const int l2 = threadIdx.x & 63, r2 = threadIdx.x >> 6;
    const int n = n0 + l2;
#pragma unroll
    for (int k = 0; k < 8; ++k) {
      const int row = k * 4 + r2, jo = jo0 + row;
      if (jo < Jp && n < d.Np) {
        const long o = (long)jo * d.Nt + d.n_off + n;
        const float v = tile[l2][row];
        if (d.dtype == VKAS_BF16) reinterpret_cast<bf16_t*>(d.out)[o] = from_f32<bf16_t>(v);
        else if (d.dtype == VKAS_F16) reinterpret_cast<f16_t*>(d.out)[o] = from_f32<f16_t>(v);
        else reinterpret_cast<float*>(d.out)[o] = v;
      }
    }
    return;
  }
  const long base = (long)lb * PM_ELEMS;
#pragma unroll
  for (int u = 0; u < PM_ELEMS / 256; ++u) {
    const long i = base + u * 256 + threadIdx.x;
    if (i >= d.total) return;
    if (d.kind == 1) {
      float v;
      if (pack_dw_elem(d.w, (int)i, d.C, d.Cp, d.mode, v)) reinterpret_cast<float*>(d.out)[i] = v;
    } else {
      long o;
      const float v = pack_conv_elem(d.w, i, d.N, d.C, d.KH, d.KW, d.Np, d.Cp, d.mode, d.n_off, d.Nt, o);
      if (d.dtype == VKAS_BF16) reinterpret_cast<bf16_t*>(d.out)[o] = from_f32<bf16_t>(v);
      else if (d.dtype == VKAS_F16) reinterpret_cast<f16_t*>(d.out)[o] = from_f32<f16_t>(v);
      else reinterpret_cast<float*>(d.out)[o] = v;
    }
  }
}

template <typename T>
__global__ void pack_conv_weight_kernel(const float* __restrict__ w, T* __restrict__ out, int N, int C, int KH, int KW,
                                        int Np, int Cp, int mode, long total, int n_off, int Nt) {
  for (long i = (long)blockIdx.x * blockDim.x + threadIdx.x; i < total; i += (long)gridDim.x * blockDim.x) {
    long o2;
    const float v2 = pack_conv_elem(w, i, N, C, KH, KW, Np, Cp, mode, n_off, Nt, o2);
    out[o2] = from_f32<T>(v2);
  }
}

__global__ void unpack_conv_wgrad_kernel(const float* __restrict__ gw, float* __restrict__ grad, int N, int C, int KH,
                                         int KW, int Np, int Cp, int accumulate, long total) {
  for (long i = (long)blockIdx.x * blockDim.x + threadIdx.x; i < total; i += (long)gridDim.x * blockDim.x) {
    long r = i;
    const int kx = (int)(r % KW); r /= KW;
    const int ky = (int)(r % KH); r /= KH;
    const int c = (int)(r % C); r /= C;
    const int n = (int)r;
    const float v = gw[(((long)n * KH + ky) * KW + kx) * Cp + c];
    grad[i] = accumulate ? grad[i] + v : v;
  }
}

__global__ void pad_vector_kernel(const float* __restrict__ v, float* __restrict__ out, int n, int np) {
  const int i = blockIdx.x * blockDim.x + threadIdx.x;
  if (i < np) out[i] = i < n ? v[i] : 0.f;
}

__global__ void pack_dw_weight_kernel(const float* __restrict__ w, float* __restrict__ out, int C, int Cp, int flip) {
  const int i = blockIdx.x * blockDim.x + threadIdx.x;
  float pv;
  if (pack_dw_elem(w, i, C, Cp, flip, pv)) out[i] = pv;
}

__global__ void unpack_dw_wgrad_kernel(const float* __restrict__ gw, float* __restrict__ grad, int C, int Cp,
                                       int accumulate) {
  const int i = blockIdx.x * blockDim.x + threadIdx.x;
  if (i >= C * 49) return;
  const int c = i / 49, tap = i - c * 49;
  const float v = gw[(long)tap * Cp + c];
  grad[i] = accumulate ? grad[i] + v : v;
}

template <typename T>
__global__ void image_to_nhwc8_kernel(const float* __restrict__ img, T* __restrict__ out, int B, int C, int H, int W) {
  const long total = (long)B * H * W;
  for (long p = (long)blockIdx.x * blockDim.x + threadIdx.x; p < total; p += (long)gridDim.x * blockDim.x) {
    const long hw = (long)H * W;
    const int b = (int)(p / hw);
    const long r = p - (long)b * hw;
    float v[8] = {0, 0, 0, 0, 0, 0, 0, 0};
    for (int c = 0; c < C; ++c) v[c] = img[((long)b * C + c) * hw + r];
    store8(out + p * 8, v);
  }
}

template <typename T>
__global__ void nhwc_to_nchw_kernel(const T* __restrict__ x, long ld, float* __restrict__ out, int B, long HW, int C) {
  const long total = (long)B * C * HW;
  for (long i = (long)blockIdx.x * blockDim.x + threadIdx.x; i < total; i += (long)gridDim.x * blockDim.x) {
    const long r = i % HW;
    const long bc = i / HW;
    const int c = (int)(bc % C);
    const long b = bc / C;
    out[i] = to_f32(x[(b * HW + r) * ld + c]);
  }
}

template <typename T>
__global__ void nchw_to_nhwc_kernel(const float* __restrict__ g, T* __restrict__ out, long ld, int B, long HW, int C,
                                    int Cp) {
  const long total = (long)B * HW * Cp;
  for (long i = (long)blockIdx.x * blockDim.x + threadIdx.x; i < total; i += (long)gridDim.x * blockDim.x) {
    const int c = (int)(i % Cp);
    const long p = i / Cp;
    const long b = p / HW;
    const long r = p - b * HW;
    const float v = c < C ? g[(b * C + c) * HW + r] : 0.f;
    out[p * ld + c] = from_f32<T>(v);
  }
}

template <typename T>
__global__ void copy_channels_kernel(const T* __restrict__ x, long ldx, T* __restrict__ y, long ldy, long M, int nvec,
                                     int accumulate) {
  const long total = M * nvec;
  for (long i = (long)blockIdx.x * blockDim.x + threadIdx.x; i < total; i += (long)gridDim.x * blockDim.x) {
    const int v = (int)(i % nvec);
    const long m = i / nvec;
    float t[8];
    load8(x + m * ldx + v * 8, t);
    if (accumulate) {
      float u[8];
      load8(y + m * ldy + v * 8, u);
#pragma unroll
      for (int k = 0; k < 8; ++k) t[k] += u[k];
    }
    store8(y + m * ldy + v * 8, t);
  }
}

template <typename T>
__global__ void copy_channel_range_kernel(const T* __restrict__ x, long ldx, int c_src, T* __restrict__ y, long ldy, int c_dst,
                                          long M, int C, int Cz) {
  const long total = M * Cz;
  for (long i = (long)blockIdx.x * blockDim.x + threadIdx.x; i < total; i += (long)gridDim.x * blockDim.x) {
    const int c = (int)(i % Cz);
    const long m = i / Cz;
    y[m * ldy + c_dst + c] = c < C ? x[m * ldx + c_src + c] : from_f32<T>(0.f);
  }
}

__global__ void softplus_fwd_kernel(const float* __restrict__ x, float* __restrict__ y, long n) {
  for (long i = (long)blockIdx.x * blockDim.x + threadIdx.x; i < n; i += (long)gridDim.x * blockDim.x) {
    const float v = x[i];
    y[i] = v > 20.f ? v : log1pf(expf(v));
  }
}
__global__ void softplus_bwd_kernel(const float* __restrict__ x, const float* __restrict__ dy, float* __restrict__ dx,
                                    long n) {
  for (long i = (long)blockIdx.x * blockDim.x + threadIdx.x; i < n; i += (long)gridDim.x * blockDim.x) {
    const float v = x[i];
    dx[i] = v > 20.f ? dy[i] : dy[i] / (1.f + expf(-v));
  }
}

static inline unsigned grid1d(long total, int bs = 256) {
  long g = vkas_cdiv(total, bs);
  if (g > 16384) g = 16384;
  if (g < 1) g = 1;
  return (unsigned)g;
}

}

extern "C" int vkas_pack_conv_weight(const float* w, void* out, int N, int C, int KH, int KW, int Np, int Cp, int mode,
                                     int dtype, void* stream) {
  VKAS_CHECK(w && out, "vkas_pack_conv_weight: null pointer");
  VKAS_CHECK(N > 0 && C > 0 && KH > 0 && KW > 0 && Np >= N && Cp >= C && Np % 8 == 0 && Cp % 8 == 0,
             "vkas_pack_conv_weight: bad dims N=%d C=%d Np=%d Cp=%d", N, C, Np, Cp);
  VKAS_CHECK(mode >= 0 && mode <= 2, "vkas_pack_conv_weight: bad mode %d", mode);
  const long total = (long)Np * KH * KW * Cp;
  VKAS_DISPATCH_DTYPE(dtype, "vkas_pack_conv_weight", {
    pack_conv_weight_kernel<T><<<grid1d(total), 256, 0, vkas_stream(stream)>>>(w, (T*)out, N, C, KH, KW, Np, Cp, mode,
                                                                              total, 0, Np);
  })
  VKAS_LAUNCH_CHECK("pack_conv_weight");
  return VKAS_OK;
}

extern "C" int vkas_pack_conv_weight_slice(const float* w, void* out, int N, int C, int KH, int KW, int Np, int Cp, int mode,
                                           int n_off, int Nt, int dtype, void* stream) {
  VKAS_CHECK(w && out, "vkas_pack_conv_weight_slice: null pointer");
  VKAS_CHECK(N > 0 && C > 0 && KH > 0 && KW > 0 && Np >= N && Cp >= C && Np % 8 == 0 && Cp % 8 == 0,
             "vkas_pack_conv_weight_slice: bad dims N=%d C=%d Np=%d Cp=%d", N, C, Np, Cp);
  VKAS_CHECK(mode == 0 || mode == 1 || mode == 3, "vkas_pack_conv_weight_slice: mode must be 0 (forward), 1 (dgrad) or 3 (rows)");
  VKAS_CHECK(n_off >= 0 && n_off % 8 == 0 && Nt % 8 == 0 && n_off + Np <= Nt, "vkas_pack_conv_weight_slice: bad slice %d + %d of %d",
             n_off, Np, Nt);
  const long total = (long)Np * KH * KW * Cp;
  VKAS_DISPATCH_DTYPE(dtype, "vkas_pack_conv_weight_slice", {
    pack_conv_weight_kernel<T><<<grid1d(total), 256, 0, vkas_stream(stream)>>>(w, (T*)out, N, C, KH, KW, Np, Cp, mode,
                                                                              total, n_off, Nt);
  })
  VKAS_LAUNCH_CHECK("pack_conv_weight_slice");
  return VKAS_OK;
}

extern "C" int vkas_unpack_conv_wgrad(const float* gw, float* grad, int N, int C, int KH, int KW, int Np, int Cp,
                                      int accumulate, void* stream) {
  VKAS_CHECK(gw && grad, "vkas_unpack_conv_wgrad: null pointer");
  VKAS_CHECK(N > 0 && C > 0 && Np >= N && Cp >= C, "vkas_unpack_conv_wgrad: bad dims");
  const long total = (long)N * C * KH * KW;
  unpack_conv_wgrad_kernel<<<grid1d(total), 256, 0, vkas_stream(stream)>>>(gw, grad, N, C, KH, KW, Np, Cp, accumulate,
                                                                          total);
  VKAS_LAUNCH_CHECK("unpack_conv_wgrad");
  return VKAS_OK;
}

extern "C" int vkas_pad_vector(const float* v, float* out, int n, int np, void* stream) {
  VKAS_CHECK(v && out && n > 0 && np >= n, "vkas_pad_vector: bad arguments");
  pad_vector_kernel<<<(unsigned)vkas_cdiv(np, 256), 256, 0, vkas_stream(stream)>>>(v, out, n, np);
  VKAS_LAUNCH_CHECK("pad_vector");
  return VKAS_OK;
}

extern "C" int vkas_pack_many_blocks(const vkas_pack_desc* d) {
  if (!d) return 0;
  if (d->kind == 0 && d->mode == 1) return (int)(vkas_cdiv((long)d->Cp * d->KH * d->KW, 32) * vkas_cdiv(d->Np, 64));
  return (int)vkas_cdiv(d->total, 2048);
}

extern "C" int vkas_pack_many(const vkas_pack_desc* descs, const int* block_start, int count, int total_blocks, void* stream) {
  VKAS_CHECK(descs && block_start && count > 0 && total_blocks > 0, "vkas_pack_many: bad arguments");
  pack_many_kernel<<<(unsigned)total_blocks, 256, 0, vkas_stream(stream)>>>(descs, block_start, count);
  VKAS_LAUNCH_CHECK("pack_many");
  return VKAS_OK;
}

extern "C" size_t vkas_dw_weight_elems(int Cp) { return (size_t)105 * (size_t)Cp; }

extern "C" int vkas_pack_dw_weight(const float* w, float* out, int C, int Cp, int flip, void* stream) {
  VKAS_CHECK(w && out && C > 0 && Cp >= C && Cp % 8 == 0, "vkas_pack_dw_weight: bad arguments");
  pack_dw_weight_kernel<<<(unsigned)vkas_cdiv(105L * Cp, 256), 256, 0, vkas_stream(stream)>>>(w, out, C, Cp, flip);
  VKAS_LAUNCH_CHECK("pack_dw_weight");
  return VKAS_OK;
}

struct AccumMany {
  const float* src[16];
  float* dst[16];
  int n[16];
};
__global__ void accumulate_many_kernel(AccumMany a) {
  const int k = blockIdx.y;
  const float* s = a.src[k];
  float* d = a.dst[k];
  for (int i = blockIdx.x * blockDim.x + threadIdx.x; i < a.n[k]; i += gridDim.x * blockDim.x) d[i] += s[i];
}

extern "C" int vkas_accumulate_many(int count, const float* const* src, float* const* dst, const int* n, void* stream) {
  VKAS_CHECK(count >= 0 && count <= 16 && (count == 0 || (src && dst && n)), "vkas_accumulate_many: bad arguments (count=%d)", count);
  if (count == 0) return VKAS_OK;
  AccumMany a;
  int nmax = 0;
  for (int k = 0; k < count; ++k) {
    VKAS_CHECK(src[k] && dst[k] && n[k] >= 0, "vkas_accumulate_many: bad vector %d", k);
    a.src[k] = src[k];
    a.dst[k] = dst[k];
    a.n[k] = n[k];
    nmax = n[k] > nmax ? n[k] : nmax;
  }
  if (nmax == 0) return VKAS_OK;
  long bx = vkas_cdiv(nmax, 256);
  if (bx > 64) bx = 64;
  accumulate_many_kernel<<<dim3((unsigned)bx, (unsigned)count), 256, 0, vkas_stream(stream)>>>(a);
  VKAS_LAUNCH_CHECK("accumulate_many");
  return VKAS_OK;
}

extern "C" int vkas_unpack_dw_wgrad(const float* gw, float* grad, int C, int Cp, int accumulate, void* stream) {
  VKAS_CHECK(gw && grad && C > 0 && Cp >= C, "vkas_unpack_dw_wgrad: bad arguments");
  unpack_dw_wgrad_kernel<<<(unsigned)vkas_cdiv(49L * C, 256), 256, 0, vkas_stream(stream)>>>(gw, grad, C, Cp, accumulate);
  VKAS_LAUNCH_CHECK("unpack_dw_wgrad");
  return VKAS_OK;
}

extern "C" int vkas_image_nchw_to_nhwc8(const float* img, void* out, int B, int C, int H, int W, int dtype,
                                        void* stream) {
  VKAS_CHECK(img && out && vkas_aligned16(out), "vkas_image_nchw_to_nhwc8: null/misaligned pointer");
  VKAS_CHECK(B >= 0 && C > 0 && C <= 8 && H > 0 && W > 0, "vkas_image_nchw_to_nhwc8: bad dims");
  if (B == 0) return VKAS_OK;
  VKAS_DISPATCH_DTYPE(dtype, "vkas_image_nchw_to_nhwc8", {
    image_to_nhwc8_kernel<T><<<grid1d((long)B * H * W), 256, 0, vkas_stream(stream)>>>(img, (T*)out, B, C, H, W);
  })
  VKAS_LAUNCH_CHECK("image_nchw_to_nhwc8");
  return VKAS_OK;
}

extern "C" int vkas_nhwc_to_nchw_f32(const void* x, long ld, float* out, int B, int H, int W, int C, int dtype,
                                     void* stream) {
  VKAS_CHECK(x && out && B >= 0 && H > 0 && W > 0 && C > 0 && ld >= C, "vkas_nhwc_to_nchw_f32: bad arguments");
  if (B == 0) return VKAS_OK;
  VKAS_DISPATCH_DTYPE(dtype, "vkas_nhwc_to_nchw_f32", {
    nhwc_to_nchw_kernel<T><<<grid1d((long)B * C * H * W), 256, 0, vkas_stream(stream)>>>((const T*)x, ld, out, B,
                                                                                        (long)H * W, C);
  })
  VKAS_LAUNCH_CHECK("nhwc_to_nchw_f32");
  return VKAS_OK;
}

extern "C" int vkas_nchw_f32_to_nhwc(const float* g, void* out, long ld, int B, int H, int W, int C, int Cp, int dtype,
                                     void* stream) {
  VKAS_CHECK(g && out && B >= 0 && H > 0 && W > 0 && C > 0 && Cp >= C && ld >= Cp, "vkas_nchw_f32_to_nhwc: bad arguments");
  if (B == 0) return VKAS_OK;
  VKAS_DISPATCH_DTYPE(dtype, "vkas_nchw_f32_to_nhwc", {
    nchw_to_nhwc_kernel<T><<<grid1d((long)B * H * W * Cp), 256, 0, vkas_stream(stream)>>>(g, (T*)out, ld, B, (long)H * W,
                                                                                         C, Cp);
  })
  VKAS_LAUNCH_CHECK("nchw_f32_to_nhwc");
  return VKAS_OK;
}

extern "C" int vkas_copy_channels(const void* x, long ldx, void* y, long ldy, long M, int Cp, int accumulate, int dtype,
                                  void* stream) {
  VKAS_CHECK(x && y && vkas_aligned16(x) && vkas_aligned16(y), "vkas_copy_channels: null/misaligned pointer");
  VKAS_CHECK(Cp > 0 && Cp % 8 == 0 && ldx >= Cp && ldy >= Cp && ldx % 8 == 0 && ldy % 8 == 0, "vkas_copy_channels: bad strides");
  if (M <= 0) return VKAS_OK;
  VKAS_DISPATCH_DTYPE(dtype, "vkas_copy_channels", {
    copy_channels_kernel<T><<<grid1d(M * (Cp / 8)), 256, 0, vkas_stream(stream)>>>((const T*)x, ldx, (T*)y, ldy, M,
                                                                                  Cp / 8, accumulate);
  })
  VKAS_LAUNCH_CHECK("copy_channels");
  return VKAS_OK;
}

extern "C" int vkas_copy_channel_range(const void* x, long ldx, int c_src, void* y, long ldy, int c_dst, long M, int C,
                                       int zero_tail, int dtype, void* stream) {
  VKAS_CHECK(x && y, "vkas_copy_channel_range: null pointer");
  VKAS_CHECK(C > 0 && zero_tail >= 0 && c_src >= 0 && c_dst >= 0 && ldx >= c_src + C && ldy >= c_dst + C + zero_tail,
             "vkas_copy_channel_range: channel range [%d, %d) / [%d, %d) outside the pixel strides %ld / %ld", c_src, c_src + C,
             c_dst, c_dst + C + zero_tail, ldx, ldy);
  if (M <= 0) return VKAS_OK;
  VKAS_DISPATCH_DTYPE(dtype, "vkas_copy_channel_range", {
    copy_channel_range_kernel<T><<<grid1d(M * (C + zero_tail)), 256, 0, vkas_stream(stream)>>>(
        (const T*)x, ldx, c_src, (T*)y, ldy, c_dst, M, C, C + zero_tail);
  })
  VKAS_LAUNCH_CHECK("copy_channel_range");
  return VKAS_OK;
}

extern "C" int vkas_softplus_fwd(const float* x, float* y, long n, void* stream) {
  VKAS_CHECK(x && y && n >= 0, "vkas_softplus_fwd: bad arguments");
  if (n == 0) return VKAS_OK;
  softplus_fwd_kernel<<<grid1d(n), 256, 0, vkas_stream(stream)>>>(x, y, n);
  VKAS_LAUNCH_CHECK("softplus_fwd");
  return VKAS_OK;
}

extern "C" int vkas_softplus_bwd(const float* x, const float* dy, float* dx, long n, void* stream) {
  VKAS_CHECK(x && dy && dx && n >= 0, "vkas_softplus_bwd: bad arguments");
  if (n == 0) return VKAS_OK;
  softplus_bwd_kernel<<<grid1d(n), 256, 0, vkas_stream(stream)>>>(x, dy, dx, n);
  VKAS_LAUNCH_CHECK("softplus_bwd");
  return VKAS_OK;
}
```

### vkit_ocr_model_adaptive_scaling_amd/ops.py

```python
import copy
import ctypes
import os
import weakref
from typing import Optional, Sequence, Tuple

import torch
from torch.autograd import Function

from . import _lib
from ._lib import lib, check, ConvGeom, Epilogue

_FLOAT = torch.float32


def rup8(c: int) -> int:
    return (c + 7) // 8 * 8


_DTYPE_CODES = {torch.float32: _lib.F32, torch.bfloat16: _lib.BF16, torch.float16: _lib.F16}
_MFMA_DTYPES = (torch.bfloat16, torch.float16)


def _dtc(dtype: torch.dtype) -> int:
    try:
# ... 12 lines not shown

def _p(t: Optional[torch.Tensor]):
    return None if t is None else ctypes.c_void_p(t.data_ptr())


def _require_cuda(*ts):
    for t in ts:
        if t is not None and not t.is_cuda:
            raise RuntimeError('vkas ops run on the MI355X only (tensor is on %s); there is no CPU fallback' % t.device)


def act_ok(t: torch.Tensor) -> bool:
    if t.dim() != 4 or t.shape[3] % 8 != 0:
        return False
    B, H, W, C = t.shape
    ld = t.stride(2) if W > 1 else (t.stride(1) if H > 1 else (t.stride(0) if B > 1 else C))
    if t.stride(3) != 1 and C > 1:
        return False
    if ld < C or ld % 8 != 0 or t.data_ptr() % 16 != 0:
        return False
    if W > 1 and t.stride(2) != ld:
        return False
    if H > 1 and t.stride(1) != W * ld:
        return False
    if B > 1 and t.stride(0) != H * W * ld:
        return False
    return True


def act_ld(t: torch.Tensor) -> int:
    B, H, W, C = t.shape
    if W > 1:
        return t.stride(2)
    if H > 1:
        return t.stride(1)
    if B > 1:
        return t.stride(0)
    return C


def as_act(t: torch.Tensor) -> torch.Tensor:
    return t if act_ok(t) else t.contiguous()


def new_act(B, H, W, Cp, like: torch.Tensor) -> torch.Tensor:
    return torch.empty((B, H, W, Cp), dtype=like.dtype, device=like.device)


def _ws(nbytes: int, device) -> torch.Tensor:
    return torch.empty(((nbytes + 3) // 4 + 4,), dtype=_FLOAT, device=device)


def _workspace(what: str, nbytes: int, device) -> torch.Tensor:
    if nbytes < 0:
        check(-1, what)
    return torch.empty((max(nbytes, 256),), dtype=torch.uint8, device=device)


class _ZeroArena:

    def __init__(self):
        self.buf: Optional[torch.Tensor] = None
        self.off = 0
        self.want = 0
        self.live = False

    def take(self, n: int, device) -> Optional[torch.Tensor]:
        n_al = -(-n // 64) * 64
        self.want += n_al
        if not self.live or self.buf.device != device or self.off + n_al > self.buf.numel():
            return None
        t = self.buf[self.off:self.off + n]
        self.off += n_al
        return t

    def reset(self):
        if self.want == 0 and self.off == 0:
            return
        if self.buf is None or self.want > self.buf.numel():
            dev = self.buf.device if self.buf is not None else torch.device('cuda', torch.cuda.current_device())
            self.buf = None
            self.buf = torch.zeros((self.want,), dtype=_FLOAT, device=dev)
        else:
            self.buf.zero_()
        self.off, self.want, self.live = 0, 0, True


_ZERO_ARENA = _ZeroArena()
_NO_ZERO_ARENA = os.environ.get('VKAS_NO_ZERO_ARENA') is not None


def zero_arena_reset():
    if not _NO_ZERO_ARENA:
        _ZERO_ARENA.reset()


def zeros_f32(n: int, device, step_scratch: bool) -> torch.Tensor:
    if step_scratch and not _NO_ZERO_ARENA:
        t = _ZERO_ARENA.take(n, device)
        if t is not None:
            return t
    return torch.zeros((n,), dtype=_FLOAT, device=device)


_PACK_CACHE = {}
_PACK_EPOCH = [0]
_PACK_PLAN = {}
_PACK_TABLE = [None]


def invalidate_packed_params():
    _PACK_EPOCH[0] += 1
    _PACK_CACHE.clear()
    _PACK_PLAN.clear()


def _plan_pack(k, descs, params):
    _PACK_PLAN[k] = (descs, tuple(weakref.ref(p) for p in params), tuple(p.data_ptr() for p in params))


def _conv_desc(w4: torch.Tensor, out: torch.Tensor, Np: int, Cp: int, mode: int, n_off: int, Nt: int, dtype) -> _lib.PackDesc:
    N, C, KH, KW = w4.shape
    return _lib.PackDesc(w4.data_ptr(), out.data_ptr(), Np * KH * KW * Cp, 0, N, C, KH, KW, Np, Cp, mode, n_off, Nt, _dtc(dtype))


def refresh_packed_params():
    _PACK_EPOCH[0] += 1
    live = {}
    for k, (descs, refs, ptrs) in _PACK_PLAN.items():
        params = [r() for r in refs]
        if k in _PACK_CACHE and all(p is not None and p.data_ptr() == q for p, q in zip(params, ptrs)):
            live[k] = (descs, refs, ptrs)
    for k in list(_PACK_CACHE):
        if k not in live:
            del _PACK_CACHE[k]
    _PACK_PLAN.clear()
    _PACK_PLAN.update(live)
    if not live:
        return
    keys = tuple(live)
    descs = [d for k in keys for d in live[k][0]]
    sig = b''.join(bytes(d) for d in descs)
    tab = _PACK_TABLE[0]
    if tab is None or tab[0] != sig:
        arr = (_lib.PackDesc * len(descs))(*descs)
        starts = [0]
        for d in descs:
            starts.append(starts[-1] + lib.vkas_pack_many_blocks(ctypes.byref(d)))
        dev = _PACK_CACHE[keys[0]][2].device
        table = torch.frombuffer(bytearray(bytes(arr)), dtype=torch.uint8).to(dev)
        tab = (sig, table, torch.tensor(starts, dtype=torch.int32, device=dev), len(descs), starts[-1])
        _PACK_TABLE[0] = tab
    check(lib.vkas_pack_many(_p(tab[1]), _p(tab[2]), tab[3], tab[4], _stream()), 'pack_many')
    for k in keys:
        stamp, refs, out = _PACK_CACHE[k]
        if isinstance(refs, tuple):
            params = [r() for r in refs]
            stamp = (tuple(p._version for p in params), _PACK_EPOCH[0], tuple(p.data_ptr() for p in params))
        else:
            src = refs()
            stamp = (src._version, _PACK_EPOCH[0], src.data_ptr())
        _PACK_CACHE[k] = (stamp, refs, out)


def _cached_pack(src: torch.Tensor, key, build):
    if not (src.is_leaf and src.requires_grad):
        return build()
    k = (id(src), key)
    ent = _PACK_CACHE.get(k)
    stamp = (src._version, _PACK_EPOCH[0], src.data_ptr())
    if ent is not None and ent[0] == stamp and ent[1]() is src:
        return ent[2]
    out = build()
    _PACK_CACHE[k] = (stamp, weakref.ref(src), out)
    return out


def pack_conv_weight(w: torch.Tensor, Np: int, Cp: int, mode: int, dtype: torch.dtype) -> torch.Tensor:
    def build():
        w4 = w if w.dim() == 4 else w.view(w.shape[0], w.shape[1], 1, 1)
        N, C, KH, KW = w4.shape
        out = torch.empty((Np * KH * KW * Cp,), dtype=dtype, device=w.device)
        check(lib.vkas_pack_conv_weight(_p(w4.contiguous()), _p(out), N, C, KH, KW, Np, Cp, mode,
                                        _dtc(dtype), _stream()), 'pack_conv_weight')
        if w.is_leaf and w.requires_grad and w4.is_contiguous():
            _plan_pack((id(w), key), [_conv_desc(w4, out, Np, Cp, mode, 0, Np, dtype)], [w])
        return out
    key = ('conv', Np, Cp, mode, dtype)
    return _cached_pack(w, key, build)


def _cached_pack_pair(a: torch.Tensor, b: torch.Tensor, key, build):
    if not (a.is_leaf and a.requires_grad and b.is_leaf and b.requires_grad):
        return build()
    k = (id(a), id(b), key)
    ent = _PACK_CACHE.get(k)
    stamp = (a._version, b._version, _PACK_EPOCH[0], a.data_ptr(), b.data_ptr())
    if ent is not None and ent[0] == stamp and ent[1]() is a and ent[3]() is b:
        return ent[2]
    out = build()
    _PACK_CACHE[k] = (stamp, weakref.ref(a), out, weakref.ref(b))
    return out


_NO_CHAIN = os.environ.get('VKAS_NO_MLP_CHAIN') is not None


_CHAIN_MAX_C = int(os.environ.get('VKAS_MLP_CHAIN_MAX_C', '384'))


def _chain_width_ok(C: int) -> bool:
    return C <= min(_CHAIN_MAX_C, 256) or (256 < C <= min(_CHAIN_MAX_C, 384) and C % 16 == 0) or (384 < C <= _CHAIN_MAX_C)


_NO_CHAIN_LN = os.environ.get('VKAS_NO_CHAIN_LN') is not None
_CHAIN_PAIR_MIN_ROWS = int(os.environ.get('VKAS_MLP_CHAIN_PAIR_MIN_ROWS', '16384'))


def mlp_chain_eligible(x: torch.Tensor, C: int) -> bool:
    if 256 < C <= 384 and x.shape[0] * x.shape[1] * x.shape[2] < _CHAIN_PAIR_MIN_ROWS:
        return False
    return (not _NO_CHAIN and x.dtype in _MFMA_DTYPES and x.shape[3] == C and _chain_width_ok(C)
            and lib.vkas_mlp_chain_image_elems(C) > 0)


def pack_mlp_chain(w1: torch.Tensor, w2: torch.Tensor, b1: Optional[torch.Tensor], C: int, mode: int,
                   dtype: torch.dtype) -> torch.Tensor:
    def build():
        img = torch.empty((lib.vkas_mlp_chain_image_elems(C),), dtype=dtype, device=w1.device)
        check(lib.vkas_mlp_chain_pack(_p(w1.contiguous()), _p(w2.contiguous()), _p(b1.contiguous()) if mode == 0 else None, C,
                                      mode, _p(img), _dtc(dtype), _stream()), 'mlp_chain_pack')
        return img
    if mode == 0:
        return _cached_pack_pair(w1, w2, ('chain', C, mode, dtype, b1._version, b1.data_ptr()), build)
    return _cached_pack_pair(w1, w2, ('chain', C, mode, dtype), build)


def pack_dw_weight(w: torch.Tensor, C: int, Cp: int, flip: int) -> torch.Tensor:
    def build():
        out = torch.empty((lib.vkas_dw_weight_elems(Cp),), dtype=_FLOAT, device=w.device)
        check(lib.vkas_pack_dw_weight(_p(w.contiguous()), _p(out), C, Cp, flip, _stream()), 'pack_dw_weight')
        if w.is_leaf and w.requires_grad and w.is_contiguous():
            _plan_pack((id(w), key), [_lib.PackDesc(w.data_ptr(), out.data_ptr(), 105 * Cp, 1, 0, C, 0, 0, 0, Cp, flip, 0, 0, 0)], [w])
        return out
    key = ('dw', C, Cp, flip)
    return _cached_pack(w, key, build)


def pad_vector(v: Optional[torch.Tensor], npad: int) -> Optional[torch.Tensor]:
    if v is None:
        return None
    if v.dim() == 1 and v.numel() == npad and v.is_contiguous():
        return v

    def build():
        flat = v.reshape(-1)
        if flat.numel() == npad and flat.is_contiguous():
            return flat
        out = torch.empty((npad,), dtype=_FLOAT, device=v.device)
        check(lib.vkas_pad_vector(_p(flat.contiguous()), _p(out), flat.numel(), npad, _stream()), 'pad_vector')
        return out
    return _cached_pack(v, ('pad', npad), build)


def _geom(B, Hin, Win, Hout, Wout, Cp, ldx, KH, KW, stride, pad) -> ConvGeom:
    return ConvGeom(B, Hin, Win, Hout, Wout, Cp, ldx, KH, KW, stride, pad)


class LaunchTimer:

    def __init__(self):
        self.records = []

    def summary(self):
        out = {}
        for kind, s, e, flops, M, N, K, _ in self.records:
            d = out.setdefault(kind, {'launches': 0, 'ms': 0.0, 'flops': 0.0})
            d['launches'] += 1
            d['ms'] += s.elapsed_time(e)
            d['flops'] += flops
        return out


TIMER: Optional[LaunchTimer] = None


def gemm_kernel_name(x, wgrad, geom, Np, lddy=0, head_width=0, flags=0, has_gb=False) -> str:
    if x.dtype not in _MFMA_DTYPES:
        return 'gemm_tn_simple' if wgrad else 'gemm_nt_simple'
    info = _lib.GemmPlanInfo()
    check(lib.vkas_conv_gemm_plan(wgrad, ctypes.byref(geom), Np, lddy, head_width, flags, int(has_gb), None, ctypes.byref(info)),
          'conv_gemm_plan')
    return info.name.decode()


def _timed(kind, x, flops, M, N, K, fn, nbytes=0.0):
    if TIMER is None:
        return fn()
    s, e = torch.cuda.Event(enable_timing=True), torch.cuda.Event(enable_timing=True)
    s.record()
    r = fn()
    e.record()
    TIMER.records.append((kind, s, e, flops, M, N, K, nbytes))
    return r


def conv_gemm(x: torch.Tensor, geom: ConvGeom, Bw: torch.Tensor, Np: int, out: torch.Tensor, mode=_lib.EPI_NONE,
              bias=None, out2=None, aux=None, colscale=None, rowscale=None, rows_per_image=0, patch=0, patch_hw=(0, 0),
              patch_Cp=0, nk=None, head=None):
    if TIMER is not None:
        M = geom.B * geom.Hout * geom.Wout
        N, K = nk if nk is not None else (Np, geom.KH * geom.KW * geom.Cp)
        kind = gemm_kernel_name(x, 0, geom, Np, head_width=max(head.np[i] for i in range(head.n_heads)) if head is not None else 0)
        es = x.element_size()
        nbytes = (geom.B * geom.Hin * geom.Win * geom.Cp + M * Np * ((out is not None) + (out2 is not None) + (aux is not None))) * es
        return _timed(kind, x, 2.0 * M * N * K, M, N, K,
                      lambda: _conv_gemm(x, geom, Bw, Np, out, mode, bias, out2, aux, colscale, rowscale, rows_per_image,
                                         patch, patch_hw, patch_Cp, head), nbytes)
    return _conv_gemm(x, geom, Bw, Np, out, mode, bias, out2, aux, colscale, rowscale, rows_per_image, patch, patch_hw,
                      patch_Cp, head)


def _conv_gemm(x, geom, Bw, Np, out, mode, bias, out2, aux, colscale, rowscale, rows_per_image, patch, patch_hw,
               patch_Cp, head=None):
    epi = Epilogue(mode, _p(bias).value if bias is not None else None, out.data_ptr() if out is not None else None,
                   act_ld(out) if out is not None else 0,
                   out2.data_ptr() if out2 is not None else None, act_ld(out2) if out2 is not None else 0,
                   aux.data_ptr() if aux is not None else None, act_ld(aux) if aux is not None else 0,
                   colscale.data_ptr() if colscale is not None else None,
                   rowscale.data_ptr() if rowscale is not None else None, rows_per_image, patch, patch_hw[0],
                   patch_hw[1], patch_Cp)
    if head is not None:
        epi.head = head
    check(lib.vkas_conv_gemm_fwd(_p(x), ctypes.byref(geom), _p(Bw), Np, ctypes.byref(epi), _dt(x), _stream()),
          'conv_gemm_fwd')
    return out


def grad_sink(param: Optional[torch.Tensor]):
    s = getattr(param, '_vkas_sink', None) if param is not None else None
    return s if s is not None and s[0].grad_view_ok(s[1]) else None


def _accumulate_pieces(pieces):
    for i in range(0, len(pieces), 16):
        part = pieces[i:i + 16]
        n = len(part)
        src = (ctypes.c_void_p * n)(*[a for a, _, _ in part])
        dst = (ctypes.c_void_p * n)(*[b for _, b, _ in part])
        cnt = (ctypes.c_int * n)(*[c for _, _, c in part])
        check(lib.vkas_accumulate_many(n, src, dst, cnt, _stream()), 'accumulate_many')


def deliver_small_grads(pairs):
    out, todo = [], []
    for param, g in pairs:
        s = grad_sink(param) if g is not None else None
        if s is None or g.dtype != _FLOAT or g.numel() != param.numel():
            out.append(g)
        else:
            todo.append((s, param, g.contiguous()))
            out.append(None)
    _accumulate_pieces([(g.data_ptr(), p.grad.data_ptr(), g.numel()) for _, p, g in todo])
    for s, _, _ in todo:
        s[0].grad_delivered(s[1])
    return out


def conv_wgrad(x: torch.Tensor, geom: ConvGeom, dy: torch.Tensor, Np: int, nk=None, with_bias: bool = False,
               x_gelu: bool = False, gw_into: Optional[torch.Tensor] = None, gb_into: Optional[torch.Tensor] = None,
               step_scratch: bool = False, ordered: bool = False):
    assert not (ordered and (with_bias or x_gelu or gw_into is not None))
    K = geom.KH * geom.KW * geom.Cp
    n_new = (0 if gw_into is not None else Np * K) + (Np if with_bias and gb_into is None else 0)
    buf = zeros_f32(n_new, x.device, step_scratch) if n_new else None
    gw = gw_into if gw_into is not None else buf[:Np * K]
    gb = None
    if with_bias:
        gb = gb_into if gb_into is not None else buf[n_new - Np:]
    M = geom.B * geom.Hout * geom.Wout

    def run():
        if ordered:
            check(lib.vkas_conv_gemm_wgrad_ordered(_p(x), ctypes.byref(geom), _p(dy), act_ld(dy), Np, _p(gw), _dt(x), _stream()),
                  'conv_gemm_wgrad_ordered')
            return gw
        fn = lib.vkas_conv_gemm_wgrad_gelu if x_gelu else lib.vkas_conv_gemm_wgrad
        check(fn(_p(x), ctypes.byref(geom), _p(dy), act_ld(dy), Np, _p(gw), _p(gb), _dt(x), _stream()), 'conv_gemm_wgrad')
        return (gw, gb) if with_bias else gw
    if TIMER is None:
        return run()
    kind = gemm_kernel_name(x, 1, geom, Np, act_ld(dy), flags=int(x_gelu) + 2 * int(ordered), has_gb=gb is not None)
    N, Kl = nk if nk is not None else (Np, K)
    nbytes = (geom.B * geom.Hin * geom.Win * geom.Cp + M * Np) * x.element_size() + 4.0 * Np * K
    return _timed(kind, x, 2.0 * M * N * Kl, M, N, Kl, run, nbytes)


def unpack_wgrad(gw: torch.Tensor, shape4, Np: int, Cp: int, into: Optional[torch.Tensor] = None) -> torch.Tensor:
    N, C, KH, KW = shape4
    g = torch.empty((N, C, KH, KW), dtype=_FLOAT, device=gw.device) if into is None else into
    check(lib.vkas_unpack_conv_wgrad(_p(gw), _p(g), N, C, KH, KW, Np, Cp, int(into is not None), _stream()),
          'unpack_conv_wgrad')
    return g


def conv_param_grads(x, geom, dy, Np: int, weight: torch.Tensor, bias: Optional[torch.Tensor], x_gelu: bool = False):
    w4 = weight if weight.dim() == 4 else weight.view(weight.shape[0], weight.shape[1], 1, 1)
    N, C, KH, KW = w4.shape
    Cp = geom.Cp
    nk = (N, C * KH * KW)
    sw, sb = grad_sink(weight), grad_sink(bias)
    same_layout = KH == 1 and KW == 1 and Np == N and Cp == C
    gw_into = weight.grad.view(-1) if (sw is not None and same_layout) else None
    gb_into = bias.grad if (sb is not None and Np == N) else None
    scratch = sw is not None and (bias is None or sb is not None)
    r = conv_wgrad(x, geom, dy, Np, nk=nk, with_bias=bias is not None, x_gelu=x_gelu, gw_into=gw_into, gb_into=gb_into,
                   step_scratch=scratch)
    gwp, gbp = r if bias is not None else (r, None)
    if gw_into is not None:
        gw = None
    elif sw is not None:
        unpack_wgrad(gwp, (N, C, KH, KW), Np, Cp, into=weight.grad.view(N, C, KH, KW))
        gw = None
    else:
        gw = unpack_wgrad(gwp, (N, C, KH, KW), Np, Cp).view(weight.shape)
    gb = None
    if bias is not None and gb_into is None:
        gb = gbp[:N].clone() if scratch else gbp[:N]
    if sw is not None:
        sw[0].grad_delivered(sw[1])
    if gb_into is not None:
        sb[0].grad_delivered(sb[1])
    return gw, gb


def colsum(y: torch.Tensor, n_logical: int) -> torch.Tensor:
    B, H, W, Np = y.shape
    M = B * H * W
    out = torch.empty((Np,), dtype=_FLOAT, device=y.device)
    nbytes = lib.vkas_colsum_ws_bytes(M, Np)
    ws = _ws(nbytes, y.device)
    check(lib.vkas_colsum(_p(y), act_ld(y), M, Np, _p(out), 0, _p(ws), nbytes, _dt(y), _stream()), 'colsum')
    return out[:n_logical]


def layernorm_fwd(x: torch.Tensor, gamma: torch.Tensor, beta: torch.Tensor, C: int, act_gelu: bool,
                  out: Optional[torch.Tensor] = None):
    B, H, W, Cp = x.shape
    M = B * H * W
    y = new_act(B, H, W, Cp, x) if out is None else out
    stats = torch.empty((M, 2), dtype=_FLOAT, device=x.device)
    gamma, beta = pad_vector(gamma, Cp), pad_vector(beta, Cp)
    check(lib.vkas_layernorm_fwd(_p(x), act_ld(x), _p(gamma), _p(beta), _p(y), act_ld(y), _p(stats), M, C, Cp,
                                 int(act_gelu), _dt(x), _stream()), 'layernorm_fwd')
    return y, stats


def layernorm_bwd(x, gamma, beta, stats, dy, C: int, act_gelu: bool, defer: bool = False):
    B, H, W, Cp = x.shape
    M = B * H * W
    dx = new_act(B, H, W, Cp, x)
    nbytes = lib.vkas_layernorm_bwd_ws_bytes(M, Cp)
    ws = _ws(nbytes, x.device)
    gamma, beta = pad_vector(gamma, Cp), pad_vector(beta, Cp)
    if defer:
        check(lib.vkas_layernorm_bwd(_p(x), act_ld(x), _p(gamma), _p(beta), _p(stats), _p(dy), act_ld(dy), _p(dx),
                                     act_ld(dx), None, None, _p(ws), nbytes, M, C, Cp, int(act_gelu), _dt(x),
                                     _stream()), 'layernorm_bwd')
        return dx, ws, lib.vkas_layernorm_bwd_parts(M, Cp)
    dgb = torch.empty((2 * Cp,), dtype=_FLOAT, device=x.device)
    dg, db = dgb[:Cp], dgb[Cp:]
    check(lib.vkas_layernorm_bwd(_p(x), act_ld(x), _p(gamma), _p(beta), _p(stats), _p(dy), act_ld(dy), _p(dx),
                                 act_ld(dx), _p(dg), _p(db), _p(ws), nbytes, M, C, Cp, int(act_gelu), _dt(x),
                                 _stream()), 'layernorm_bwd')
    return dx, dg[:C], db[:C]


_NO_FINALIZE_MANY = os.environ.get('VKAS_NO_FINALIZE_MANY') is not None


def finalize_many(items):
    for i in range(0, len(items), 8):
        part = items[i:i + 8]
        n = len(part)
        src = (ctypes.c_void_p * n)(*[ws.data_ptr() + 4 * col for ws, col, _, _, _, _, _ in part])
        P = (ctypes.c_long * n)(*[p for _, _, p, _, _, _, _ in part])
        nn = (ctypes.c_int * n)(*[c for _, _, _, c, _, _, _ in part])
        ld = (ctypes.c_int * n)(*[l for _, _, _, _, l, _, _ in part])
        dst = (ctypes.c_void_p * n)(*[o.data_ptr() for _, _, _, _, _, o, _ in part])
        acc = (ctypes.c_int * n)(*[int(a) for _, _, _, _, _, _, a in part])
        check(lib.vkas_finalize_many(n, src, P, nn, ld, dst, acc, _stream()), 'finalize_many')


def small_grad_views(params, Cp: int):
    if _NO_FINALIZE_MANY:
        return None
    sinks = [grad_sink(p) for p in params]
    if any(s is None for s in sinks):
        return None
    if any(p.numel() != Cp or not p.grad.is_contiguous() or p.grad.dtype != _FLOAT for p in params):
        return None
    return sinks


def resize_fwd(x, size: Tuple[int, int], mode: int, out=None, accumulate=False):
    B, Hin, Win, Cp = x.shape
    Hout, Wout = size
    y = new_act(B, Hout, Wout, Cp, x) if out is None else out
    nbytes = B * Cp * x.element_size() * (Hin * Win + Hout * Wout * (2 if accumulate else 1))
    x2 = mode == 0 and Hout == 2 * Hin and Wout == 2 * Win and Hin > 1 and Win > 1
    _timed('resize2x_fwd_kernel' if x2 else 'resize_fwd_kernel', x, 0.0, B * Hout * Wout, Cp, 0,
           lambda: check(lib.vkas_resize_fwd(_p(x), act_ld(x), _p(y), act_ld(y), B, Hin, Win, Hout, Wout, Cp, mode,
                                             int(accumulate), _dt(x), _stream()), 'resize_fwd'), nbytes)
    return y


def resize_bwd(dy, in_size: Tuple[int, int], mode: int):
    B, Hout, Wout, Cp = dy.shape
    Hin, Win = in_size
    dx = new_act(B, Hin, Win, Cp, dy)
    nbytes = B * Cp * dy.element_size() * (Hin * Win + Hout * Wout)
    x2 = mode == 0 and Hout == 2 * Hin and Wout == 2 * Win and Hin > 1 and Win > 1
    wsb = lib.vkas_resize_bwd_ws_bytes(B, Hin, Win, Hout, Wout, Cp)
    ws = _ws(wsb, dy.device) if wsb else None
    name = 'resize2x_bwd_kernel' if x2 else ('resize_bwd_x+y_kernel' if wsb else 'resize_bwd_kernel')
    _timed(name, dy, 0.0, B * Hout * Wout, Cp, 0,
           lambda: check(lib.vkas_resize_bwd_ws(_p(dy), act_ld(dy), _p(dx), act_ld(dx), _p(ws), wsb, B, Hin, Win, Hout, Wout, Cp,
                                                mode, 0, _dt(dy), _stream()), 'resize_bwd'), nbytes)
    return dx


def copy_channels(x, out, accumulate=False):
    B, H, W, Cp = x.shape
    check(lib.vkas_copy_channels(_p(x), act_ld(x), _p(out), act_ld(out), B * H * W, Cp, int(accumulate), _dt(x),
                                 _stream()), 'copy_channels')
    return out


class ImageToAct(Function):

    @staticmethod
    def forward(ctx, img: torch.Tensor, dtype: torch.dtype):
        _require_cuda(img)
        if img.dtype != _FLOAT:
            img = img.float()
        img = img.contiguous()
        B, C, H, W = img.shape
        out = torch.empty((B, H, W, 8), dtype=dtype, device=img.device)
        check(lib.vkas_image_nchw_to_nhwc8(_p(img), _p(out), B, C, H, W,
                                           _dtc(dtype), _stream()),
              'image_nchw_to_nhwc8')
        ctx.C = C
        return out

    @staticmethod
    def backward(ctx, g):
        if not ctx.needs_input_grad[0]:
            return None, None
        g = as_act(g)
        B, H, W, Cp = g.shape
        out = torch.empty((B, ctx.C, H, W), dtype=_FLOAT, device=g.device)
        check(lib.vkas_nhwc_to_nchw_f32(_p(g), act_ld(g), _p(out), B, H, W, ctx.C, _dt(g), _stream()), 'nhwc_to_nchw_f32')
        return out, None


def images_to_act(imgs: Sequence[torch.Tensor], dtype: torch.dtype) -> torch.Tensor:
    if any(i.requires_grad for i in imgs) and torch.is_grad_enabled():
        return ImageToAct.apply(torch.cat(list(imgs), 0), dtype)
    _require_cuda(*imgs)
    H, W = imgs[0].shape[2], imgs[0].shape[3]
    out = torch.empty((sum(i.shape[0] for i in imgs), H, W, 8), dtype=dtype, device=imgs[0].device)
    b0 = 0
    for img in imgs:
        if img.dim() != 4 or img.shape[2:] != (H, W):
            raise ValueError('images_to_act: the batches must share their spatial size')
        img = img.detach()
        img = (img if img.dtype == _FLOAT else img.float()).contiguous()
        B, C = img.shape[0], img.shape[1]
        check(lib.vkas_image_nchw_to_nhwc8(_p(img), _p(out[b0:b0 + B]), B, C, H, W, _dtc(dtype), _stream()),
              'image_nchw_to_nhwc8')
        b0 += B
    return out


class Conv(Function):

    @staticmethod
    def forward(ctx, x, weight, bias, stride: int, pad: int, need_input_grad: bool = True):
        _require_cuda(x, weight)
        x = as_act(x)
        w4 = weight if weight.dim() == 4 else weight.view(weight.shape[0], weight.shape[1], 1, 1)
        N, C, KH, KW = w4.shape
        B, Hin, Win, Cp = x.shape
        if Cp != rup8(C):
            raise ValueError(f'Conv: activation has {Cp} (padded) channels, weight expects {C}')
        Hout = (Hin + 2 * pad - KH) // stride + 1
        Wout = (Win + 2 * pad - KW) // stride + 1
        Np = rup8(N)
        Bw = pack_conv_weight(weight, Np, Cp, 0, x.dtype)
        out = new_act(B, Hout, Wout, Np, x)
        geom = _geom(B, Hin, Win, Hout, Wout, Cp, act_ld(x), KH, KW, stride, pad)
        conv_gemm(x, geom, Bw, Np, out, _lib.EPI_NONE, bias=pad_vector(bias, Np), nk=(N, C * KH * KW))
        ctx.save_for_backward(x, weight, bias if bias is not None else torch.empty(0, device=x.device))
        ctx.cfg = (stride, pad, bias is not None, need_input_grad)
        return out

    @staticmethod
    def backward(ctx, dy):
        x, weight, bias = ctx.saved_tensors
        stride, pad, has_bias, need_input_grad = ctx.cfg
        dy = as_act(dy)
        w4 = weight if weight.dim() == 4 else weight.view(weight.shape[0], weight.shape[1], 1, 1)
        N, C, KH, KW = w4.shape
        B, Hin, Win, Cp = x.shape
        _, Hout, Wout, Np = dy.shape
        geom = _geom(B, Hin, Win, Hout, Wout, Cp, act_ld(x), KH, KW, stride, pad)
        gw, gb = conv_param_grads(x, geom, dy, Np, weight, bias if has_bias else None)
        dx = None
        if need_input_grad and ctx.needs_input_grad[0]:
            if stride == 1:
                Bt = pack_conv_weight(weight, Np, Cp, 1, x.dtype)
                dx = new_act(B, Hin, Win, Cp, x)
                g2 = _geom(B, Hout, Wout, Hin, Win, Np, act_ld(dy), KH, KW, 1, KH - 1 - pad)
                conv_gemm(dy, g2, Bt, Cp, dx, _lib.EPI_NONE, nk=(C, N * KH * KW))
            else:
                assert stride == KH == KW and pad == 0
                Bt = pack_conv_weight(weight, Np, Cp, 2, x.dtype)
                full = (Hout * stride == Hin and Wout * stride == Win)
                dx = new_act(B, Hin, Win, Cp, x) if full else torch.zeros_like(x, memory_format=torch.contiguous_format)
                g2 = _geom(B, Hout, Wout, Hout, Wout, Np, act_ld(dy), 1, 1, 1, 0)
                conv_gemm(dy, g2, Bt, KH * KW * Cp, dx, _lib.EPI_PATCH, patch=KH, patch_hw=(Hout, Wout), patch_Cp=Cp,
                          nk=(C * KH * KW, N))
        return dx, gw, gb, None, None, None


def pack_upconv5_weight(w: torch.Tensor, f: int, Np: int, Cp: int, transposed: int, dtype: torch.dtype) -> torch.Tensor:
    def build():
        N, C = w.shape[0], w.shape[1]
        out = torch.empty((lib.vkas_upconv5_fold_elems(Np, Cp, f, transposed),), dtype=dtype, device=w.device)
        check(lib.vkas_upconv5_fold(_p(w.contiguous()), _p(out), N, C, Np, Cp, f, transposed, _dtc(dtype), _stream()),
              'upconv5_fold')
        return out
    return _cached_pack(w, ('upconv5', f, Np, Cp, transposed, dtype), build)

# ... 674 lines not shown

def pass_point_sparse(src: torch.Tensor, dst: torch.Tensor) -> torch.Tensor:
    pts = point_mark(src)
    if pts is not None:
        point_sparse(dst, pts[0], pts[1])
    return dst


def _point_sparse_run(dprojs, B, H, W):
    marks = [point_mark(d) for d in dprojs]
    idx = [h for h, m in enumerate(marks) if m is not None]
    if not idx:
        return None
    h0, h1 = idx[0], idx[-1] + 1
    py, px = marks[h0]
    if idx != list(range(h0, h1)) or (h0 > 0 and h1 < len(dprojs)):
        return None
    if any(m[0] is not py or m[1] is not px for m in (marks[h] for h in idx)):
        return None
    if (py.dim() != 2 or py.shape != px.shape or py.shape[0] != B or py.dtype != torch.int64 or px.dtype != torch.int64
            or not py.is_cuda or not py.is_contiguous() or not px.is_contiguous() or py.shape[1] == 0):
        return None
    if py.numel() * 16 > B * H * W:
        return None
    return h0, h1, py, px


class ConvNextLayer(Function):

    @staticmethod
    def forward(ctx, x, dw_w, dw_b, ln_g, ln_b, w1, b1, w2, b2, block_scale, rowscale, keep: bool = True):
        _require_cuda(x, dw_w)
        x = as_act(x)
        B, H, W, Cp = x.shape
        C = dw_w.shape[0]
        M = B * H * W
        dt, st = _dt(x), _stream()
        wdw = pack_dw_weight(dw_w, C, Cp, 0)
        y = new_act(B, H, W, Cp, x)
        dwb = pad_vector(dw_b, Cp)
        dw_fwd_name = 'dwconv7x7_mfma_kernel' if x.dtype in _MFMA_DTYPES else 'dwconv7x7_fwd_kernel'
        _timed(dw_fwd_name, x, 2.0 * 49 * M * C, M, Cp, 49,
               lambda: check(lib.vkas_dwconv7x7_fwd(_p(x), act_ld(x), _p(wdw), _p(dwb), None, 0, _p(y), Cp, B, H, W, Cp, dt,
                                                    st), 'dwconv7x7_fwd'), 2.0 * M * Cp * x.element_size())
        C4 = w1.shape[0]
        C4p = rup8(C4)
        chain = C4 == 4 * C and mlp_chain_eligible(x, C)
        fuse_ln = chain and not _NO_CHAIN_LN
        if not fuse_ln:
            yn, stats = layernorm_fwd(y, ln_g.contiguous(), ln_b.contiguous(), C, False)
        out = new_act(B, H, W, Cp, x)
        z = new_act(B, H, W, Cp, x)
        cs = pad_vector(block_scale, Cp)
        rs = None if rowscale is None else rowscale.to(_FLOAT).contiguous()
        if chain and fuse_ln:
            h = new_act(B, H, W, C4p, x) if keep else None
            yn = new_act(B, H, W, Cp, x) if keep else None
            stats = torch.empty((M, 2), dtype=_FLOAT, device=x.device) if keep else None
            if not keep:
                z = None
            g = None
            img = pack_mlp_chain(w1, w2, b1, C, 0, x.dtype)
            es = x.element_size()
            lg, lb = pad_vector(ln_g.contiguous(), Cp), pad_vector(ln_b.contiguous(), Cp)
            _timed('mlp_chain_pair_kernel<fwd>' if 256 < C <= 384 else 'mlp_chain_kernel<fwd>', x, 4.0 * M * C * C4, M, C, C4,
                   lambda: check(lib.vkas_mlp_chain_ln_fwd(_p(y), Cp, _p(lg), _p(lb), _p(yn), Cp, _p(stats), _p(img),
                                                           _p(pad_vector(b2, Cp)), _p(x), act_ld(x), _p(cs), _p(rs), H * W,
                                                           _p(h), C4p, _p(z), Cp, _p(out), Cp, M, C, dt, st),
                                 'mlp_chain_ln_fwd'),
                   float(M) * ((5 * Cp + C4p) if keep else 3 * Cp) * es)
            if not keep:
                return out
        elif chain:
            h = new_act(B, H, W, C4p, x) if keep else None
            if not keep:
                z = None
            g = None
            img = pack_mlp_chain(w1, w2, b1, C, 0, x.dtype)
            es = x.element_size()
            _timed('mlp_chain_pair_kernel<fwd>' if 256 < C <= 384 else 'mlp_chain_kernel<fwd>', x, 4.0 * M * C * C4, M, C, C4,
                   lambda: check(lib.vkas_mlp_chain_fwd(_p(yn), Cp, _p(img), _p(pad_vector(b2, Cp)),
                                                        _p(x), act_ld(x), _p(cs), _p(rs), H * W, _p(h), C4p, _p(z), Cp,
                                                        _p(out), Cp, M, C, dt, st), 'mlp_chain_fwd'),
                   float(M) * ((4 * Cp + C4p) if keep else 3 * Cp) * es)
            if not keep:
                return out
        else:
            h = new_act(B, H, W, C4p, x) if keep else None
            if not keep:
                z = None
            g = new_act(B, H, W, C4p, x)
            g1 = _geom(B, H, W, H, W, Cp, Cp, 1, 1, 1, 0)
            conv_gemm(yn, g1, pack_conv_weight(w1, C4p, Cp, 0, x.dtype), C4p, h, _lib.EPI_GELU, bias=pad_vector(b1, C4p),
                      out2=g)
            g2 = _geom(B, H, W, H, W, C4p, C4p, 1, 1, 1, 0)
            conv_gemm(g, g2, pack_conv_weight(w2, Cp, C4p, 0, x.dtype), Cp, out, _lib.EPI_SCALE_RES,
                      bias=pad_vector(b2, Cp), out2=z, aux=x, colscale=cs, rowscale=rs, rows_per_image=H * W)
            if not keep:
                return out
        empty = torch.empty(0, device=x.device)
        ctx.save_for_backward(x, y, stats, yn, h, g if g is not None else empty, z, dw_w, ln_g, ln_b, w1, w2, block_scale,
                              rs if rs is not None else empty, b1, dw_b, b2)
        ctx.chain = chain
        ctx.has_rs = rs is not None
        return out

    @staticmethod
    def backward(ctx, dout):
        x, y, stats, yn, h, g, z, dw_w, ln_g, ln_b, w1, w2, block_scale, rs, b1, dw_b, b2 = ctx.saved_tensors
        rs = rs if ctx.has_rs else None
        dout = as_act(dout)
        B, H, W, Cp = x.shape
        C = dw_w.shape[0]
        C4 = w1.shape[0]
        C4p = rup8(C4)
        M = B * H * W
        dt, st, dev = _dt(x), _stream(), x.device
        cs = pad_vector(block_scale, Cp)
        sinks = small_grad_views((block_scale, b2, ln_g, ln_b, dw_b), Cp)
        dz = new_act(B, H, W, Cp, x)
        nbytes = lib.vkas_scale_res_bwd_ws_bytes(M, Cp)
        ws_sr = _ws(nbytes, dev)
        if sinks is None:
            dsb = torch.empty((2 * Cp,), dtype=_FLOAT, device=dev)
            dscale, db2 = dsb[:Cp], dsb[Cp:]
        else:
            dscale = db2 = None
        check(lib.vkas_scale_res_bwd(_p(dout), act_ld(dout), _p(z), Cp, _p(cs), _p(rs), H * W, _p(dz), Cp, _p(dscale),
                                     _p(db2), _p(ws_sr), nbytes, M, Cp, dt, st), 'scale_res_bwd')
        g2 = _geom(B, H, W, H, W, C4p, C4p, 1, 1, 1, 0)
        g1 = _geom(B, H, W, H, W, Cp, Cp, 1, 1, 1, 0)
        if ctx.chain:
            dh = new_act(B, H, W, C4p, x)
            dyn = new_act(B, H, W, Cp, x)
            imgt = pack_mlp_chain(w1, w2, None, C, 1, x.dtype)
            _timed('mlp_chain_pair_kernel<bwd>' if 256 < C <= 384 else 'mlp_chain_kernel<bwd>', x, 4.0 * M * C * C4, M, C, C4,
                   lambda: check(lib.vkas_mlp_chain_bwd(_p(dz), Cp, _p(imgt), _p(h), C4p, _p(dh), C4p, _p(dyn), Cp, M, C,
                                                        dt, st), 'mlp_chain_bwd'),
                   float(M) * (2 * Cp + 2 * C4p) * x.element_size())
            gw2, _ = conv_param_grads(h, g2, dz, Cp, w2, None, x_gelu=True)
        else:
            gw2, _ = conv_param_grads(g, g2, dz, Cp, w2, None)
            dh = new_act(B, H, W, C4p, x)
            conv_gemm(dz, g1, pack_conv_weight(w2, Cp, C4p, 1, x.dtype), C4p, dh, _lib.EPI_DGELU, aux=h)
        gw1, db1 = conv_param_grads(yn, g1, dh, C4p, w1, b1)
        if not ctx.chain:
            dyn = new_act(B, H, W, Cp, x)
            conv_gemm(dh, g2, pack_conv_weight(w1, C4p, Cp, 1, x.dtype), Cp, dyn, _lib.EPI_NONE)
        if sinks is None:
            dy, dlg, dlb = layernorm_bwd(y, ln_g.contiguous(), ln_b.contiguous(), stats, dyn, C, False)
        else:
            dy, ws_ln, parts_ln = layernorm_bwd(y, ln_g.contiguous(), ln_b.contiguous(), stats, dyn, C, False, defer=True)
            dlg = dlb = None
        gdwb = torch.empty((50 * Cp,), dtype=_FLOAT, device=dev)
        gdw, gdb = gdwb[:49 * Cp], gdwb[49 * Cp:]
        nbytes = lib.vkas_dwconv7x7_wgrad_ws_bytes(B, H, W, Cp)
        ws = _ws(nbytes, dev)
        mfma = x.dtype in _MFMA_DTYPES
        _timed('dwconv7x7_wgrad_mfma_kernel' if mfma else 'dwconv7x7_wgrad_kernel', x, 2.0 * 49 * M * C, M, Cp, 49,
               lambda: check(lib.vkas_dwconv7x7_wgrad(_p(x), act_ld(x), _p(dy), Cp, _p(gdw) if sinks is None else None,
                                                      _p(gdb) if sinks is None else None, _p(ws), nbytes, B, H, W,
                                                      Cp, dt, st), 'dwconv7x7_wgrad'), 2.0 * M * Cp * x.element_size())
        if sinks is not None:
            p_sr = lib.vkas_scale_res_bwd_parts(M, Cp)
            p_dw = lib.vkas_dwconv7x7_wgrad_parts(B, H, W, Cp, dt)
            finalize_many([(ws_sr, 0, p_sr, Cp, 2 * Cp, block_scale.grad, True), (ws_sr, Cp, p_sr, Cp, 2 * Cp, b2.grad, True),
                           (ws_ln, 0, parts_ln, Cp, 2 * Cp, ln_g.grad, True), (ws_ln, Cp, parts_ln, Cp, 2 * Cp, ln_b.grad, True),
                           (ws, 0, p_dw, 49 * Cp, 50 * Cp, gdw, False), (ws, 49 * Cp, p_dw, Cp, 50 * Cp, dw_b.grad, True)])
            for sk in sinks:
                sk[0].grad_delivered(sk[1])
        sdw = grad_sink(dw_w)
        if sdw is not None:
            check(lib.vkas_unpack_dw_wgrad(_p(gdw), _p(dw_w.grad), C, Cp, 1, st), 'unpack_dw_wgrad')
            sdw[0].grad_delivered(sdw[1])
            gdw_ref = None
        else:
            gdw_ref = torch.empty((C, 1, 7, 7), dtype=_FLOAT, device=dev)
            check(lib.vkas_unpack_dw_wgrad(_p(gdw), _p(gdw_ref), C, Cp, 0, st), 'unpack_dw_wgrad')
        dx = None
        if ctx.needs_input_grad[0]:
            wflip = pack_dw_weight(dw_w, C, Cp, 1)
            dx = new_act(B, H, W, Cp, x)
            _timed('dwconv7x7_mfma_kernel' if mfma else 'dwconv7x7_fwd_kernel', x, 2.0 * 49 * M * C, M, Cp, 49,
                   lambda: check(lib.vkas_dwconv7x7_fwd(_p(dy), Cp, _p(wflip), None, _p(dout), act_ld(dout), _p(dx), Cp, B, H,
                                                        W, Cp, dt, st), 'dwconv7x7_dgrad'), 3.0 * M * Cp * x.element_size())
        if sinks is not None:
            return (dx, gdw_ref, None, None, None, gw1, db1, gw2, None, None, None, None)
        gdb_, dlg, dlb, db2_, dsc = deliver_small_grads([(dw_b, gdb[:C]), (ln_g, dlg), (ln_b, dlb), (b2, db2[:C]),
                                                         (block_scale, dscale[:C].view(block_scale.shape))])
        return (dx, gdw_ref, gdb_, dlg, dlb, gw1, db1, gw2, db2_, dsc, None, None)


class Resize(Function):

    @staticmethod
    def forward(ctx, x, size, mode: int):
        _require_cuda(x)
        x = as_act(x)
        ctx.in_size = (x.shape[1], x.shape[2])
        ctx.mode = mode
        return resize_fwd(x, tuple(size), mode)

    @staticmethod
    def backward(ctx, dy):
        return resize_bwd(as_act(dy), ctx.in_size, ctx.mode), None, None


class ResizeAdd(Function):

    @staticmethod
    def forward(ctx, dst, src, mode: int):
        _require_cuda(dst, src)
        if not act_ok(dst):
            raise ValueError('ResizeAdd: dst must be a valid NHWC activation')
        src = as_act(src)
        ctx.in_size = (src.shape[1], src.shape[2])
        ctx.mode = mode
        resize_fwd(src, (dst.shape[1], dst.shape[2]), mode, out=dst, accumulate=True)
        ctx.mark_dirty(dst)
        return dst

    @staticmethod
    def backward(ctx, dy):
        dy = as_act(dy)
        return dy, resize_bwd(dy, ctx.in_size, ctx.mode), None


class AdaptiveAvgPool(Function):

    @staticmethod
    def forward(ctx, x, s: int):
        _require_cuda(x)
        x = as_act(x)
        B, H, W, Cp = x.shape
        y = new_act(B, s, s, Cp, x)
        check(lib.vkas_adaptive_avgpool_fwd(_p(x), act_ld(x), _p(y), Cp, B, H, W, s, Cp, _dt(x), _stream()),
              'adaptive_avgpool_fwd')
        ctx.cfg = (H, W, s)
        return y

    @staticmethod
    def backward(ctx, dy):
        H, W, s = ctx.cfg
        dy = as_act(dy)
        B, _, _, Cp = dy.shape
        dx = new_act(B, H, W, Cp, dy)
        check(lib.vkas_adaptive_avgpool_bwd(_p(dy), act_ld(dy), _p(dx), Cp, B, H, W, s, Cp, 0, _dt(dy), _stream()),
              'adaptive_avgpool_bwd')
        return dx, None


class AdaptiveAvgPools(Function):

    @staticmethod
    def forward(ctx, x, *scales: int):
        _require_cuda(x)
        x = as_act(x)
        B, H, W, Cp = x.shape
        ys = []
        for s in scales:
            y = new_act(B, s, s, Cp, x)
            check(lib.vkas_adaptive_avgpool_fwd(_p(x), act_ld(x), _p(y), Cp, B, H, W, s, Cp, _dt(x), _stream()),
                  'adaptive_avgpool_fwd')
            ys.append(y)
        ctx.cfg = (B, H, W, Cp, tuple(scales), x.dtype, x.device)
        return tuple(ys)

    @staticmethod
    def backward(ctx, *dys):
        B, H, W, Cp, scales, dtype, dev = ctx.cfg
        dx = torch.empty((B, H, W, Cp), dtype=dtype, device=dev)
        first = True
        for s, dy in zip(scales, dys):
            if dy is None:
                continue
            dy = as_act(dy)
            check(lib.vkas_adaptive_avgpool_bwd(_p(dy), act_ld(dy), _p(dx), Cp, B, H, W, s, Cp, 0 if first else 1, _dt(dy),
                                                _stream()), 'adaptive_avgpool_bwd')
            first = False
        if first:
            dx.zero_()
        return (dx,) + (None,) * len(scales)


class Cat(Function):

    @staticmethod
    def forward(ctx, *parts):
        _require_cuda(*parts)
        parts = [as_act(p) for p in parts]
        B, H, W, _ = parts[0].shape
        widths = [p.shape[3] for p in parts]
        out = new_act(B, H, W, sum(widths), parts[0])
        off = 0
        for p, w in zip(parts, widths):
            copy_channels(p, out[..., off:off + w])
            off += w
        ctx.widths = widths
        return out

    @staticmethod
    def backward(ctx, dy):
        dy = as_act(dy)
        outs, off = [], 0
        for w in ctx.widths:
            outs.append(dy[..., off:off + w])
            off += w
        return tuple(outs)


def copy_channel_range(x, c_src: int, out, c_dst: int, C: int, zero_tail: int = 0):
    B, H, W, _ = x.shape
    check(lib.vkas_copy_channel_range(_p(x), act_ld(x), c_src, _p(out), act_ld(out), c_dst, B * H * W, C, zero_tail, _dt(x),
                                      _stream()), 'copy_channel_range')
    return out


class ResizeCat(Function):

    @staticmethod
    def forward(ctx, mode: int, widths, first, *others):
        _require_cuda(first, *others)
        first = as_act(first)
        others = [as_act(p) for p in others]
        B, H, W, w0 = first.shape
# ... 1198 lines not shown
```

Before: 315.4.

## Batch chain-image packs, fuse dw wgrad unpack into finalize, add per-pixel layout kernels

MLP chain weight images can now be repacked through the batched pack_many launch, using a new descriptor kind, instead of one kernel per image. The depthwise 7x7 weight-gradient finalize writes straight into the parameter grad in (C,49) order, which removes a separate unpack launch and scratch buffer. New per-pixel NHWC<->NCHW conversion kernels handle the C<=8 case with vectorized 16-byte loads and stores. The cost is extra complexity in the pack cache, including re-keying entries, and a layout-changing path inside the finalize kernel.

Result: no change. 316.1, median of 5 (+0.2%).

```diff
diff --git a/include/vkas.h b/include/vkas.h
--- a/include/vkas.h
+++ b/include/vkas.h
@@ -65,6 +65,8 @@
 int vkas_accumulate_many(int count, const float* const* src, float* const* dst, const int* n, void* stream);
 int vkas_finalize_many(int count, const float* const* partial, const long* P, const int* n, const int* ldp,
                        float* const* out, const int* accumulate, void* stream);
+int vkas_finalize_many_dw(int count, const float* const* partial, const long* P, const int* n, const int* ldp,
+                          float* const* out, const int* accumulate, const int* dw_C, const int* dw_Cp, void* stream);
 long vkas_layernorm_bwd_parts(long M, int Cp);
 long vkas_scale_res_bwd_parts(long M, int Cp);
 long vkas_dwconv7x7_wgrad_parts(int B, int H, int W, int Cp, int dtype);
@@ -281,6 +283,8 @@
   void* out;
   long total;
   int kind, N, C, KH, KW, Np, Cp, mode, n_off, Nt, dtype;
+  const float* w2;
+  const float* b1;
 } vkas_pack_desc;
 int vkas_pack_many(const vkas_pack_desc* descs, const int* block_start, int count, int total_blocks, void* stream);
 int vkas_pack_many_blocks(const vkas_pack_desc* d);
diff --git a/vkit_ocr_model_adaptive_scaling_amd/_lib.py b/vkit_ocr_model_adaptive_scaling_amd/_lib.py
--- a/vkit_ocr_model_adaptive_scaling_amd/_lib.py
+++ b/vkit_ocr_model_adaptive_scaling_amd/_lib.py
@@ -46,7 +46,7 @@
 class PackDesc(Structure):
     _fields_ = [('w', c_void_p), ('out', c_void_p), ('total', c_long), ('kind', c_int), ('N', c_int), ('C', c_int),
                 ('KH', c_int), ('KW', c_int), ('Np', c_int), ('Cp', c_int), ('mode', c_int), ('n_off', c_int),
-                ('Nt', c_int), ('dtype', c_int)]
+                ('Nt', c_int), ('dtype', c_int), ('w2', c_void_p), ('b1', c_void_p)]
 
 
 class RoughLossCfg(Structure):
@@ -86,6 +86,8 @@
     'vkas_accumulate_many': (c_int, [c_int, POINTER(c_void_p), POINTER(c_void_p), POINTER(c_int), _P]),
     'vkas_finalize_many': (c_int, [c_int, POINTER(c_void_p), POINTER(c_long), POINTER(c_int), POINTER(c_int), POINTER(c_void_p),
                                    POINTER(c_int), _P]),
+    'vkas_finalize_many_dw': (c_int, [c_int, POINTER(c_void_p), POINTER(c_long), POINTER(c_int), POINTER(c_int), POINTER(c_void_p),
+                                      POINTER(c_int), POINTER(c_int), POINTER(c_int), _P]),
     'vkas_layernorm_bwd_parts': (c_long, [c_long, c_int]),
     'vkas_scale_res_bwd_parts': (c_long, [c_long, c_int]),
     'vkas_dwconv7x7_wgrad_parts': (c_long, [c_int, c_int, c_int, c_int, c_int]),
diff --git a/vkit_ocr_model_adaptive_scaling_amd/csrc/chain_image.h b/vkit_ocr_model_adaptive_scaling_amd/csrc/chain_image.h
--- /dev/null
+++ b/vkit_ocr_model_adaptive_scaling_amd/csrc/chain_image.h
@@ -0,0 +1,57 @@
+#pragma once
+
+#include "vkas_common.h"
+
+__host__ __device__ constexpr int chain_ka(int KS) { return ((KS + 1) / 2) * 64; }
+__host__ __device__ constexpr int chain_img_elems(int KS) { return 32 * chain_ka(KS) + KS * 32 * 32 + 512; }
+
+__host__ __device__ inline int chain_ks(int C) {
+  if (C <= 0 || C % 8 != 0 || C > 512) return 0;
+  const int ks = (C + 31) / 32;
+  return ks <= 4 ? ks : (ks <= 6 ? 6 : (ks <= 8 ? 8 : (ks <= 12 ? 12 : 16)));
+}
+
+static inline long chain_img_pieces(int C, int KS) { return (long)(4 * C / 32) * (chain_img_elems(KS) / 8); }
+
+template <typename T>
+__device__ __forceinline__ void chain_pack_piece(const float* __restrict__ w1, const float* __restrict__ w2,
+                                                 const float* __restrict__ b1, int C, int HID, int KS, int mode,
+                                                 T* __restrict__ img, long idx) {
+  const int KA = chain_ka(KS);
+  const int pieces = chain_img_elems(KS) / 8;
+  const int j = (int)(idx / pieces);
+  int p = (int)(idx - (long)j * pieces);
+  float v[8];
+  const int a_pieces = 32 * KA / 8;
+  const int b_pieces = KS * 32 * 32 / 8;
+  if (p >= a_pieces + b_pieces) {
+    const int q = p - a_pieces - b_pieces;
+    float4 bv = make_float4(0.f, 0.f, 0.f, 0.f);
+    if (q < 8 && mode == 0 && b1) bv = *reinterpret_cast<const float4*>(b1 + j * 32 + q * 4);
+    *reinterpret_cast<float4*>(img + idx * 8) = bv;
+    return;
+  }
+  if (p < a_pieces) {
+    const int s = p / 256, rem = p - s * 256;
+    const int h = rem >> 3, cpos = rem & 7;
+    const int c = cpos ^ (h & 7);
+    const int k0 = s * 64 + c * 8;
+    const int hid = j * 32 + h;
+#pragma unroll
+    for (int i = 0; i < 8; ++i) {
+      const int k = k0 + i;
+      v[i] = k < C ? (mode == 0 ? w1[(long)hid * C + k] : w2[(long)k * HID + hid]) : 0.f;
+    }
+  } else {
+    p -= a_pieces;
+    const int R = p >> 3, cpos = p & 7;
+    const int c = cpos ^ (R & 7);
+    const int n = R * 2 + (c >> 2), g = c & 3;
+#pragma unroll
+    for (int q = 0; q < 8; ++q) {
+      const int hid = j * 32 + (q >> 2) * 16 + g * 4 + (q & 3);
+      v[q] = n < C ? (mode == 0 ? w2[(long)n * HID + hid] : w1[(long)hid * C + n]) : 0.f;
+    }
+  }
+  store8(img + idx * 8, v);
+}
diff --git a/vkit_ocr_model_adaptive_scaling_amd/csrc/gemm_api.hip b/vkit_ocr_model_adaptive_scaling_amd/csrc/gemm_api.hip
--- a/vkit_ocr_model_adaptive_scaling_amd/csrc/gemm_api.hip
+++ b/vkit_ocr_model_adaptive_scaling_amd/csrc/gemm_api.hip
@@ -236,6 +236,7 @@
   float* out[8];
   long P[8];
   int n[8], ldp[8], accumulate[8], first[9];
+  int dw_C[8], dw_Cp[8];
 };
 __global__ __launch_bounds__(256) void vkas_finalize_many_kernel(FinalizeMany a) {
   __shared__ float red[16][17];
@@ -265,13 +266,20 @@
 #pragma unroll
     for (int r = 0; r < 16; ++r) s += red[r][cl];
     float* out = a.out[k];
-    out[c] = a.accumulate[k] ? out[c] + s : s;
-  }
-}
-
-extern "C" int vkas_finalize_many(int count, const float* const* partial, const long* P, const int* n, const int* ldp,
-                                  float* const* out, const int* accumulate, void* stream) {
-  VKAS_CHECK(count >= 0 && count <= 8 && (count == 0 || (partial && P && n && ldp && out && accumulate)),
+    int o = c;
+    if (a.dw_Cp[k] > 0) {
+      const int tap = c / a.dw_Cp[k], ch = c - tap * a.dw_Cp[k];
+      if (ch >= a.dw_C[k]) return;
+      o = ch * 49 + tap;
+    }
+    out[o] = a.accumulate[k] ? out[o] + s : s;
+  }
+}
+
+extern "C" int vkas_finalize_many_dw(int count, const float* const* partial, const long* P, const int* n, const int* ldp,
+                                     float* const* out, const int* accumulate, const int* dw_C, const int* dw_Cp,
+                                     void* stream) {
+  VKAS_CHECK(count >= 0 && count <= 8 && (count == 0 || (partial && P && n && ldp && out && accumulate)) && !dw_C == !dw_Cp,
              "vkas_finalize_many: bad arguments (count=%d)", count);
   if (count == 0) return VKAS_OK;
   FinalizeMany a;
@@ -286,9 +294,14 @@
       a.n[k] = n[k];
       a.ldp[k] = ldp[k];
       a.accumulate[k] = accumulate[k];
+      a.dw_C[k] = dw_Cp ? dw_C[k] : 0;
+      a.dw_Cp[k] = dw_Cp ? dw_Cp[k] : 0;
+      VKAS_CHECK(a.dw_Cp[k] == 0 || (a.dw_C[k] > 0 && a.dw_C[k] <= a.dw_Cp[k] && n[k] == 49 * a.dw_Cp[k]),
+                 "vkas_finalize_many: reduction %d: a depthwise output takes 49 * Cp columns, 0 < C <= Cp", k);
       blocks += (int)vkas_cdiv(n[k], 16);
     } else {
       a.partial[k] = nullptr; a.out[k] = nullptr; a.P[k] = 0; a.n[k] = 0; a.ldp[k] = 0; a.accumulate[k] = 0;
+      a.dw_C[k] = 0; a.dw_Cp[k] = 0;
     }
   }
   a.first[8] = blocks;
@@ -297,6 +310,11 @@
   vkas_finalize_many_kernel<<<(unsigned)blocks, 256, 0, vkas_stream(stream)>>>(a);
   VKAS_LAUNCH_CHECK("finalize_many");
   return VKAS_OK;
+}
+
+extern "C" int vkas_finalize_many(int count, const float* const* partial, const long* P, const int* n, const int* ldp,
+                                  float* const* out, const int* accumulate, void* stream) {
+  return vkas_finalize_many_dw(count, partial, P, n, ldp, out, accumulate, nullptr, nullptr, stream);
 }
 
 int vkas_colreduce_finalize(const float* partial, long P, int n, int ldp, float* out, int accumulate,
diff --git a/vkit_ocr_model_adaptive_scaling_amd/csrc/mlp_chain.hip b/vkit_ocr_model_adaptive_scaling_amd/csrc/mlp_chain.hip
--- a/vkit_ocr_model_adaptive_scaling_amd/csrc/mlp_chain.hip
+++ b/vkit_ocr_model_adaptive_scaling_amd/csrc/mlp_chain.hip
@@ -2,6 +2,7 @@
 
 #include <type_traits>
 
+#include "chain_image.h"
 #include "vkas_common.h"
 
 namespace {
@@ -14,9 +15,6 @@
 #define CHAIN_ABL 0
 #endif
 constexpr int ABL = CHAIN_ABL;
-
-__host__ __device__ constexpr int chain_ka(int KS) { return ((KS + 1) / 2) * 64; }
-__host__ __device__ constexpr int chain_img_elems(int KS) { return 32 * chain_ka(KS) + KS * 32 * 32 + 512; }
 
 template <typename T, typename V4>
 __device__ __forceinline__ V4 chain_gelu4(const V4& h) {
@@ -37,46 +35,9 @@
 template <typename T>
 __global__ void mlp_chain_pack_kernel(const float* __restrict__ w1, const float* __restrict__ w2,
                                       const float* __restrict__ b1, int C, int HID, int KS, int mode, T* __restrict__ img) {
-  const int KA = chain_ka(KS);
-  const int pieces = chain_img_elems(KS) / 8;
   const long idx = (long)blockIdx.x * blockDim.x + threadIdx.x;
-  const int nchunks = HID / 32;
-  if (idx >= (long)nchunks * pieces) return;
-  const int j = (int)(idx / pieces);
-  int p = (int)(idx - (long)j * pieces);
-  float v[8];
-  const int a_pieces = 32 * KA / 8;
-  const int b_pieces = KS * 32 * 32 / 8;
-  if (p >= a_pieces + b_pieces) {
-    const int q = p - a_pieces - b_pieces;
-    float4 bv = make_float4(0.f, 0.f, 0.f, 0.f);
-    if (q < 8 && mode == 0 && b1) bv = *reinterpret_cast<const float4*>(b1 + j * 32 + q * 4);
-    *reinterpret_cast<float4*>(img + idx * 8) = bv;
-    return;
-  }
-  if (p < a_pieces) {
-    const int s = p / 256, rem = p - s * 256;
-    const int h = rem >> 3, cpos = rem & 7;
-    const int c = cpos ^ (h & 7);
-    const int k0 = s * 64 + c * 8;
-    const int hid = j * 32 + h;
-#pragma unroll
-    for (int i = 0; i < 8; ++i) {
-      const int k = k0 + i;
-      v[i] = k < C ? (mode == 0 ? w1[(long)hid * C + k] : w2[(long)k * HID + hid]) : 0.f;
-    }
-  } else {
-    p -= a_pieces;
-    const int R = p >> 3, cpos = p & 7;
-    const int c = cpos ^ (R & 7);
-    const int n = R * 2 + (c >> 2), g = c & 3;
-#pragma unroll
-    for (int q = 0; q < 8; ++q) {
-      const int hid = j * 32 + (q >> 2) * 16 + g * 4 + (q & 3);
-      v[q] = n < C ? (mode == 0 ? w2[(long)n * HID + hid] : w1[(long)hid * C + n]) : 0.f;
-    }
-  }
-  store8(img + idx * 8, v);
+  if (idx >= (long)(HID / 32) * (chain_img_elems(KS) / 8)) return;
+  chain_pack_piece<T>(w1, w2, b1, C, HID, KS, mode, img, idx);
 }
 
 struct ChainArgs {
@@ -983,12 +944,6 @@
   }
 }
 
-static int chain_ks(int C) {
-  if (C <= 0 || C % 8 != 0 || C > 512) return 0;
-  const int ks = (C + 31) / 32;
-  return ks <= 4 ? ks : (ks <= 6 ? 6 : (ks <= 8 ? 8 : (ks <= 12 ? 12 : 16)));
-}
-
 static int chain_pair_mode() {
   static const int mode = [] {
     const char* v = getenv("VKAS_CHAIN_PAIR");
@@ -1045,7 +1000,7 @@
   VKAS_CHECK(ks > 0, "vkas_mlp_chain_pack: C=%d is not covered (multiple of 8, <= 512)", C);
   VKAS_CHECK(mode == 0 || mode == 1, "vkas_mlp_chain_pack: mode must be 0 (forward) or 1 (backward)");
   VKAS_CHECK(dtype == VKAS_BF16 || dtype == VKAS_F16, "vkas_mlp_chain_pack: 16-bit storage types only");
-  const long pieces = (long)(4 * C / 32) * (chain_img_elems(ks) / 8);
+  const long pieces = chain_img_pieces(C, ks);
   if (dtype == VKAS_BF16)
     mlp_chain_pack_kernel<bf16_t><<<(unsigned)vkas_cdiv(pieces, 256), 256, 0, vkas_stream(stream)>>>(w1, w2, b1, C, 4 * C, ks,
                                                                                                      mode, (bf16_t*)img);
diff --git a/vkit_ocr_model_adaptive_scaling_amd/csrc/pack.hip b/vkit_ocr_model_adaptive_scaling_amd/csrc/pack.hip
--- a/vkit_ocr_model_adaptive_scaling_amd/csrc/pack.hip
+++ b/vkit_ocr_model_adaptive_scaling_amd/csrc/pack.hip
@@ -1,3 +1,4 @@
+#include "chain_image.h"
 #include "vkas_common.h"
 
 namespace {
@@ -97,6 +98,15 @@
     }
     return;
   }
+  if (d.kind == 2) {
+    const long idx = (long)lb * (PM_ELEMS / 8) + threadIdx.x;
+    if (idx * 8 >= d.total) return;
+    if (d.dtype == VKAS_BF16)
+      chain_pack_piece<bf16_t>(d.w, d.w2, d.b1, d.C, 4 * d.C, chain_ks(d.C), d.mode, reinterpret_cast<bf16_t*>(d.out), idx);
+    else
+      chain_pack_piece<f16_t>(d.w, d.w2, d.b1, d.C, 4 * d.C, chain_ks(d.C), d.mode, reinterpret_cast<f16_t*>(d.out), idx);
+    return;
+  }
   const long base = (long)lb * PM_ELEMS;
 #pragma unroll
   for (int u = 0; u < PM_ELEMS / 256; ++u) {
@@ -198,6 +208,33 @@
 }
 
 template <typename T>
+__global__ __launch_bounds__(256) void nhwc_to_nchw_px_kernel(const T* __restrict__ x, long ld, float* __restrict__ out, int B,
+                                                              long HW, int C) {
+  const long total = (long)B * HW;
+  for (long p = (long)blockIdx.x * blockDim.x + threadIdx.x; p < total; p += (long)gridDim.x * blockDim.x) {
+    const long b = p / HW, r = p - b * HW;
+    float t[8];
+    load8(x + p * ld, t);
+#pragma unroll
+    for (int c = 0; c < 8; ++c)
+      if (c < C) out[(b * C + c) * HW + r] = t[c];
+  }
+}
+
+template <typename T>
+__global__ __launch_bounds__(256) void nchw_to_nhwc_px_kernel(const float* __restrict__ g, T* __restrict__ out, long ld, int B,
+                                                              long HW, int C) {
+  const long total = (long)B * HW;
+  for (long p = (long)blockIdx.x * blockDim.x + threadIdx.x; p < total; p += (long)gridDim.x * blockDim.x) {
+    const long b = p / HW, r = p - b * HW;
+    float t[8];
+#pragma unroll
+    for (int c = 0; c < 8; ++c) t[c] = c < C ? g[(b * C + c) * HW + r] : 0.f;
+    store8(out + p * ld, t);
+  }
+}
+
+template <typename T>
 __global__ void copy_channels_kernel(const T* __restrict__ x, long ldx, T* __restrict__ y, long ldy, long M, int nvec,
                                      int accumulate) {
   const long total = M * nvec;
@@ -377,6 +414,14 @@
                                      void* stream) {
   VKAS_CHECK(x && out && B >= 0 && H > 0 && W > 0 && C > 0 && ld >= C, "vkas_nhwc_to_nchw_f32: bad arguments");
   if (B == 0) return VKAS_OK;
+  const long HW = (long)H * W;
+  if (C <= 8 && ld % 8 == 0 && vkas_aligned16(x)) {
+    VKAS_DISPATCH_DTYPE(dtype, "vkas_nhwc_to_nchw_f32", {
+      nhwc_to_nchw_px_kernel<T><<<grid1d((long)B * HW), 256, 0, vkas_stream(stream)>>>((const T*)x, ld, out, B, HW, C);
+    })
+    VKAS_LAUNCH_CHECK("nhwc_to_nchw_f32");
+    return VKAS_OK;
+  }
   VKAS_DISPATCH_DTYPE(dtype, "vkas_nhwc_to_nchw_f32", {
     nhwc_to_nchw_kernel<T><<<grid1d((long)B * C * H * W), 256, 0, vkas_stream(stream)>>>((const T*)x, ld, out, B,
                                                                                         (long)H * W, C);
@@ -389,6 +434,14 @@
                                      void* stream) {
   VKAS_CHECK(g && out && B >= 0 && H > 0 && W > 0 && C > 0 && Cp >= C && ld >= Cp, "vkas_nchw_f32_to_nhwc: bad arguments");
   if (B == 0) return VKAS_OK;
+  const long HW = (long)H * W;
+  if (Cp == 8 && ld % 8 == 0 && vkas_aligned16(out)) {
+    VKAS_DISPATCH_DTYPE(dtype, "vkas_nchw_f32_to_nhwc", {
+      nchw_to_nhwc_px_kernel<T><<<grid1d((long)B * HW), 256, 0, vkas_stream(stream)>>>(g, (T*)out, ld, B, HW, C);
+    })
+    VKAS_LAUNCH_CHECK("nchw_f32_to_nhwc");
+    return VKAS_OK;
+  }
   VKAS_DISPATCH_DTYPE(dtype, "vkas_nchw_f32_to_nhwc", {
     nchw_to_nhwc_kernel<T><<<grid1d((long)B * H * W * Cp), 256, 0, vkas_stream(stream)>>>(g, (T*)out, ld, B, (long)H * W,
                                                                                          C, Cp);
diff --git a/vkit_ocr_model_adaptive_scaling_amd/ops.py b/vkit_ocr_model_adaptive_scaling_amd/ops.py
--- a/vkit_ocr_model_adaptive_scaling_amd/ops.py
+++ b/vkit_ocr_model_adaptive_scaling_amd/ops.py
@@ -188,8 +188,22 @@
         tab = (sig, table, torch.tensor(starts, dtype=torch.int32, device=dev), len(descs), starts[-1])
         _PACK_TABLE[0] = tab
     check(lib.vkas_pack_many(_p(tab[1]), _p(tab[2]), tab[3], tab[4], _stream()), 'pack_many')
+    renamed = {}
     for k in keys:
-        stamp, refs, out = _PACK_CACHE[k]
+        ent = _PACK_CACHE[k]
+        if len(ent) == 4:
+            a, b = ent[1](), ent[3]()
+            stamp = (a._version, b._version, _PACK_EPOCH[0], a.data_ptr(), b.data_ptr())
+            del _PACK_CACHE[k]
+            k2 = _chain_rekey(k, [r() for r in live[k][1]])
+            if k2 != k:
+                if k2 in live:
+                    del _PACK_PLAN[k]
+                    continue
+                renamed[k] = k2
+            _PACK_CACHE[k2] = (stamp, ent[1], ent[2], ent[3])
+            continue
+        stamp, refs, out = ent
         if isinstance(refs, tuple):
             params = [r() for r in refs]
             stamp = (tuple(p._version for p in params), _PACK_EPOCH[0], tuple(p.data_ptr() for p in params))
@@ -197,6 +211,10 @@
             src = refs()
             stamp = (src._version, _PACK_EPOCH[0], src.data_ptr())
         _PACK_CACHE[k] = (stamp, refs, out)
+    if renamed:
+        plan = {renamed.get(k, k): v for k, v in _PACK_PLAN.items()}
+        _PACK_PLAN.clear()
+        _PACK_PLAN.update(plan)
 
 
 def _cached_pack(src: torch.Tensor, key, build):
@@ -229,7 +247,7 @@
 def _cached_pack_pair(a: torch.Tensor, b: torch.Tensor, key, build):
     if not (a.is_leaf and a.requires_grad and b.is_leaf and b.requires_grad):
         return build()
-    k = (id(a), id(b), key)
+    k = ((id(a), id(b)), key)
     ent = _PACK_CACHE.get(k)
     stamp = (a._version, b._version, _PACK_EPOCH[0], a.data_ptr(), b.data_ptr())
     if ent is not None and ent[0] == stamp and ent[1]() is a and ent[3]() is b:
@@ -260,16 +278,39 @@
             and lib.vkas_mlp_chain_image_elems(C) > 0)
 
 
+def chain_pack_desc(w1_ptr: int, w2_ptr: int, b1_ptr: Optional[int], out_ptr: int, total: int, C: int, mode: int,
+                    dtype_code: int) -> _lib.PackDesc:
+    if mode not in (0, 1):
+        raise ValueError(f'chain image mode must be 0 (forward) or 1 (backward), not {mode}')
+    if (mode == 0) != bool(b1_ptr):
+        raise ValueError('the forward chain image takes b1, the backward image does not')
+    if total <= 0 or total % 8 != 0 or out_ptr % 16 != 0:
+        raise ValueError('a chain image is a 16-byte aligned whole number of 16-byte pieces')
+    return _lib.PackDesc(w1_ptr, out_ptr, total, 2, 0, C, 0, 0, 0, 0, mode, 0, 0, dtype_code, w2_ptr, b1_ptr if mode == 0 else None)
+
+
+def _chain_key(C: int, mode: int, dtype, b1: Optional[torch.Tensor]):
+    return ('chain', C, mode, dtype, b1._version, b1.data_ptr()) if mode == 0 else ('chain', C, mode, dtype)
+
+
+def _chain_rekey(k, params):
+    ids, key = k
+    return (ids, _chain_key(key[1], key[2], key[3], params[2] if key[2] == 0 else None))
+
+
 def pack_mlp_chain(w1: torch.Tensor, w2: torch.Tensor, b1: Optional[torch.Tensor], C: int, mode: int,
                    dtype: torch.dtype) -> torch.Tensor:
     def build():
-        img = torch.empty((lib.vkas_mlp_chain_image_elems(C),), dtype=dtype, device=w1.device)
+        img = torch.empty((lib.vkas_mlp_chain_image_elems(C),), dtype=torch.int16, device=w1.device)
         check(lib.vkas_mlp_chain_pack(_p(w1.contiguous()), _p(w2.contiguous()), _p(b1.contiguous()) if mode == 0 else None, C,
                                       mode, _p(img), _dtc(dtype), _stream()), 'mlp_chain_pack')
+        srcs = [w1, w2] + ([b1] if mode == 0 else [])
+        if all(t.is_leaf and t.requires_grad and t.is_contiguous() for t in srcs):
+            _plan_pack(((id(w1), id(w2)), key), [chain_pack_desc(w1.data_ptr(), w2.data_ptr(), b1.data_ptr() if mode == 0 else None,
+                                                                 img.data_ptr(), img.numel(), C, mode, _dtc(dtype))], srcs)
         return img
-    if mode == 0:
-        return _cached_pack_pair(w1, w2, ('chain', C, mode, dtype, b1._version, b1.data_ptr()), build)
-    return _cached_pack_pair(w1, w2, ('chain', C, mode, dtype), build)
+    key = _chain_key(C, mode, dtype, b1)
+    return _cached_pack_pair(w1, w2, key, build)
 
 
 def pack_dw_weight(w: torch.Tensor, C: int, Cp: int, flip: int) -> torch.Tensor:
@@ -513,19 +554,25 @@
 
 
 _NO_FINALIZE_MANY = os.environ.get('VKAS_NO_FINALIZE_MANY') is not None
+_NO_FINALIZE_DW = os.environ.get('VKAS_NO_FINALIZE_DW') is not None
 
 
 def finalize_many(items):
     for i in range(0, len(items), 8):
         part = items[i:i + 8]
         n = len(part)
-        src = (ctypes.c_void_p * n)(*[ws.data_ptr() + 4 * col for ws, col, _, _, _, _, _ in part])
-        P = (ctypes.c_long * n)(*[p for _, _, p, _, _, _, _ in part])
-        nn = (ctypes.c_int * n)(*[c for _, _, _, c, _, _, _ in part])
-        ld = (ctypes.c_int * n)(*[l for _, _, _, _, l, _, _ in part])
-        dst = (ctypes.c_void_p * n)(*[o.data_ptr() for _, _, _, _, _, o, _ in part])
-        acc = (ctypes.c_int * n)(*[int(a) for _, _, _, _, _, _, a in part])
-        check(lib.vkas_finalize_many(n, src, P, nn, ld, dst, acc, _stream()), 'finalize_many')
+        src = (ctypes.c_void_p * n)(*[it[0].data_ptr() + 4 * it[1] for it in part])
+        P = (ctypes.c_long * n)(*[it[2] for it in part])
+        nn = (ctypes.c_int * n)(*[it[3] for it in part])
+        ld = (ctypes.c_int * n)(*[it[4] for it in part])
+        dst = (ctypes.c_void_p * n)(*[it[5].data_ptr() for it in part])
+        acc = (ctypes.c_int * n)(*[int(it[6]) for it in part])
+        if any(len(it) > 7 for it in part):
+            dwc = (ctypes.c_int * n)(*[it[7][0] if len(it) > 7 else 0 for it in part])
+            dwp = (ctypes.c_int * n)(*[it[7][1] if len(it) > 7 else 0 for it in part])
+            check(lib.vkas_finalize_many_dw(n, src, P, nn, ld, dst, acc, dwc, dwp, _stream()), 'finalize_many')
+        else:
+            check(lib.vkas_finalize_many(n, src, P, nn, ld, dst, acc, _stream()), 'finalize_many')
 
 
 def small_grad_views(params, Cp: int):
@@ -1506,8 +1553,12 @@
         else:
             dy, ws_ln, parts_ln = layernorm_bwd(y, ln_g.contiguous(), ln_b.contiguous(), stats, dyn, C, False, defer=True)
             dlg = dlb = None
-        gdwb = torch.empty((50 * Cp,), dtype=_FLOAT, device=dev)
-        gdw, gdb = gdwb[:49 * Cp], gdwb[49 * Cp:]
+        sdw = grad_sink(dw_w)
+        dw_direct = (sinks is not None and sdw is not None and not _NO_FINALIZE_DW and dw_w.grad.is_contiguous()
+                     and dw_w.grad.dtype == _FLOAT)
+        if not dw_direct:
+            gdwb = torch.empty((50 * Cp,), dtype=_FLOAT, device=dev)
+            gdw, gdb = gdwb[:49 * Cp], gdwb[49 * Cp:]
         nbytes = lib.vkas_dwconv7x7_wgrad_ws_bytes(B, H, W, Cp)
         ws = _ws(nbytes, dev)
         mfma = x.dtype in _MFMA_DTYPES
@@ -1520,11 +1571,14 @@
             p_dw = lib.vkas_dwconv7x7_wgrad_parts(B, H, W, Cp, dt)
             finalize_many([(ws_sr, 0, p_sr, Cp, 2 * Cp, block_scale.grad, True), (ws_sr, Cp, p_sr, Cp, 2 * Cp, b2.grad, True),
                            (ws_ln, 0, parts_ln, Cp, 2 * Cp, ln_g.grad, True), (ws_ln, Cp, parts_ln, Cp, 2 * Cp, ln_b.grad, True),
+                           (ws, 0, p_dw, 49 * Cp, 50 * Cp, dw_w.grad, True, (C, Cp)) if dw_direct else
                            (ws, 0, p_dw, 49 * Cp, 50 * Cp, gdw, False), (ws, 49 * Cp, p_dw, Cp, 50 * Cp, dw_b.grad, True)])
             for sk in sinks:
                 sk[0].grad_delivered(sk[1])
-        sdw = grad_sink(dw_w)
-        if sdw is not None:
+        if dw_direct:
+            sdw[0].grad_delivered(sdw[1])
+            gdw_ref = None
+        elif sdw is not None:
             check(lib.vkas_unpack_dw_wgrad(_p(gdw), _p(dw_w.grad), C, Cp, 1, st), 'unpack_dw_wgrad')
             sdw[0].grad_delivered(sdw[1])
             gdw_ref = None
```
